# liupei101/AdvMIL

Hardware: AMD Instinct MI355X
Metric: WSI bags/sec (full G+D step) (higher is better)
Workload: dtype bf16x3 (fp32 operands split hi+lo, 3 bf16 MFMAs per product, fp32 accumulate; fp32 storage); 1 GPU; ABMIL+AdvMIL(RLIP prj discriminator), 8192-patch x 1024 fp32 bags (BASELINE.json configs[1] shape; fp32 storage, bf16x3 split arithmetic: >= the bf16 the config names, within 2e-5 of the fp32 reference); gen_updates=1, distinct_resident_bags_per_gpu=64, parallelism=bag-parallel dp1, dropout=shipped rates, launch=hipGraph replay (4 captured bag groups)

## Files before the change

### advmil_amd/_lib.py

```python
import ctypes
import os
from ctypes import c_float, c_int, c_int32, c_int64, c_size_t, c_uint64, c_void_p

LIB_PATH = os.environ.get("ADVMIL_HIP_LIB") or os.path.join(os.path.dirname(os.path.abspath(__file__)), "libadvmil_hip.so")


class HipLibraryMissing(RuntimeError):
    pass


class AdvmilHipError(RuntimeError):
    pass


class Epilogue(ctypes.Structure):
    _fields_ = [("bias", c_void_p), ("act0", c_int), ("act1", c_int), ("act_split", c_int), ("drop_p", c_float),
                ("seed", c_void_p), ("stream_id", c_uint64), ("rowv", c_void_p), ("colv", c_void_p), ("rowseg", c_void_p),
                ("maskref", c_void_p), ("ldmask", c_int), ("mask_scale", c_float), ("accumulate", c_int),
                ("alpha", c_float), ("a_hi", c_void_p), ("a_lo", c_void_p), ("b_hi", c_void_p), ("b_lo", c_void_p),
                ("c_hi", c_void_p), ("c_lo", c_void_p), ("gate_wc", c_void_p), ("gate_out", c_void_p), ("gate_np", c_int),
                ("rng_row", c_void_p), ("c2", c_void_p), ("ldc2", c_int64), ("n_split", c_int64), ("bias2", c_void_p), ("colsum", c_void_p), ("maskbits", c_void_p), ("ldbits", c_int64),
                ("gate_bits_a", c_void_p), ("gate_bits_b", c_void_p), ("ldgbits", c_int64), ("c_rows_pair32", c_int)]


class DenseLayer(ctypes.Structure):
    _fields_ = [("W", c_void_p), ("bias", c_void_p), ("dW", c_void_p), ("dbias", c_void_p), ("y", c_void_p), ("K", c_int), ("N", c_int),
                ("act", c_int), ("drop_p", c_float), ("stream_id", c_uint64)]


TAIL_MAXL = 3


class DTail(ctypes.Structure):
    _fields_ = [("B", c_int), ("nx", c_int), ("ny", c_int), ("prj_src", c_int), ("xin", c_void_p), ("tin", c_void_p),
                ("x", DenseLayer * TAIL_MAXL), ("y", DenseLayer * TAIL_MAXL), ("u", c_void_p), ("w_prj", c_void_p), ("b_prj", c_void_p),
                ("dw_prj", c_void_p), ("db_prj", c_void_p), ("seed", c_void_p), ("rng_row", c_void_p), ("out", c_void_p),
                ("dout", c_void_p), ("dxin", c_void_p), ("dtin", c_void_p), ("du", c_void_p)]


class GemmTnCall(ctypes.Structure):
    _fields_ = [("M", c_int64), ("N", c_int64), ("K", c_int64), ("A", c_void_p), ("lda", c_int64), ("B", c_void_p), ("ldb", c_int64),
                ("C", c_void_p), ("ldc", c_int64), ("accumulate", ctypes.c_int32)]


class GHead(ctypes.Structure):
    _fields_ = [("B", ctypes.c_int32), ("d0", ctypes.c_int32), ("d1", ctypes.c_int32), ("d2", ctypes.c_int32), ("noise_mode", ctypes.c_int32),
                ("out_act", ctypes.c_int32), ("x", c_void_p), ("ldx", c_int64), ("Wr", c_void_p), ("br", c_void_p), ("W0", c_void_p),
                ("b0", c_void_p), ("W1", c_void_p), ("b1", c_void_p), ("p1", c_float), ("p2", c_float), ("seed", c_void_p),
                ("sid1", c_uint64), ("sid2", c_uint64), ("sid_noise", c_uint64), ("rng_row", c_void_p), ("noise", c_void_p),
                ("hs", c_void_p), ("h2", c_void_p), ("pred", c_void_p), ("dpred", c_void_p), ("dx", c_void_p), ("lddx", c_int64),
                ("dWr", c_void_p), ("dbr", c_void_p), ("dW0", c_void_p), ("db0", c_void_p), ("dW1", c_void_p), ("db1", c_void_p),
                ("ws", c_void_p), ("ws_bytes", c_size_t)]


SIGNATURES = {
    "advmil_version": (c_int, []),
    "advmil_gemm_f32_workspace_bytes": (c_size_t, [c_int64, c_int64, c_int]),
    "advmil_gemm_f32": (c_int, [c_int, c_int, c_int64, c_int64, c_int64, c_void_p, c_int64, c_void_p, c_int64, c_void_p,
                                c_int64, ctypes.POINTER(Epilogue), c_int, c_void_p, c_size_t, c_void_p]),
    "advmil_split_planes": (c_int, [c_void_p, c_int64, c_void_p, c_void_p, c_void_p]),
    "advmil_stage_bag": (c_int, [c_void_p, c_void_p, c_size_t, c_void_p, c_void_p, c_void_p, c_void_p, c_size_t, c_void_p]),
    "advmil_gate_interleave": (c_int, [c_void_p, c_void_p, c_void_p, c_void_p, c_int, c_void_p, c_void_p, c_void_p, c_void_p, c_int, c_void_p]),
    "advmil_gate_partial_sum": (c_int, [c_void_p, c_int, c_void_p, c_int64, c_void_p, c_void_p]),
    "advmil_gemm_f32_gate_blocks": (c_int, [c_int, c_int64]),
    "advmil_gemm_f32_colsum_rows": (c_int64, [c_int, c_int64, c_int64]),
    "advmil_merge_partials": (c_int, [c_void_p, c_int, c_int64, c_int64, c_void_p, c_int, c_void_p]),
    "advmil_set_gemm_mode": (c_int, [c_int]),
    "advmil_get_gemm_mode": (c_int, []),
    "advmil_gemm_f32_plan": (c_int, [c_int64, c_int64, c_int64, ctypes.POINTER(c_int), ctypes.POINTER(c_int)]),
    "advmil_gemm_f32_plan_layout": (c_int, [c_int, c_int, c_int64, c_int64, c_int64, ctypes.POINTER(c_int), ctypes.POINTER(c_int)]),
    "advmil_gemm_f32_plan_planes": (c_int, [c_int, c_int, c_int64, c_int64, c_int64, ctypes.POINTER(c_int)]),
    "advmil_gemm_f32_plan_tn_planes": (c_int, [c_int64, c_int64, c_int64, ctypes.POINTER(c_int), ctypes.POINTER(c_int)]),
    "advmil_gemm_f32_tiled": (c_int, [c_int, c_int, c_int64, c_int64, c_int64, c_void_p, c_int64, c_void_p, c_int64, c_void_p,
                                      c_int64, ctypes.POINTER(Epilogue), c_int, c_int, c_void_p, c_size_t, c_void_p]),
    "advmil_mha_fwd": (c_int, [c_void_p, c_void_p, c_int64, c_int, c_int, c_int, c_void_p, c_int64, c_float, c_void_p, c_uint64,
                               c_void_p, c_void_p, c_void_p, c_void_p]),
    "advmil_mha_fwd_lse": (c_int, [c_void_p, c_void_p, c_int64, c_int, c_int, c_int, c_void_p, c_int64, c_float, c_void_p, c_uint64,
                                   c_void_p, c_void_p, c_void_p, c_void_p]),
    "advmil_mha_bwd_workspace_bytes": (c_size_t, [c_int64, c_int, c_int]),
    "advmil_mha_bwd": (c_int, [c_void_p, c_void_p, c_void_p, c_void_p, c_void_p, c_int64, c_int, c_int, c_int, c_void_p, c_int64,
                               c_float, c_void_p, c_uint64, c_void_p, c_void_p, c_void_p, c_size_t, c_void_p]),
    "advmil_mha_bwd1_workspace_bytes": (c_size_t, [c_int64, c_int, c_int, c_int64]),
    "advmil_mha_bwd1": (c_int, [c_void_p, c_void_p, c_void_p, c_void_p, c_void_p, c_int64, c_int, c_int, c_int, c_void_p, c_int64,
                                c_float, c_void_p, c_uint64, c_void_p, c_void_p, c_void_p, c_size_t, c_void_p]),
    "advmil_add_dropout_ln_fwd": (c_int, [c_void_p, c_void_p, c_void_p, c_void_p, c_float, c_int64, c_int64, c_float, c_void_p,
                                          c_uint64, c_void_p, c_void_p, c_void_p, c_void_p, c_void_p, c_void_p, c_void_p, c_void_p]),
    "advmil_add_dropout_ln_bwd_workspace_bytes": (c_size_t, [c_int64, c_int64]),
    "advmil_add_dropout_ln_bwd": (c_int, [c_void_p, c_void_p, c_void_p, c_void_p, c_void_p, c_int64, c_int64, c_float, c_void_p,
                                          c_uint64, c_void_p, c_void_p, c_void_p, c_void_p, c_void_p, c_int, c_void_p, c_size_t,
                                          c_void_p]),
    "advmil_gate_score_fwd": (c_int, [c_void_p, c_void_p, c_void_p, c_float, c_void_p, c_uint64, c_uint64, c_int64, c_int64,
                                      c_void_p, c_void_p, c_void_p]),
    "advmil_softmax_pool_workspace_bytes": (c_size_t, [c_int64, c_int64, c_int]),
    "advmil_softmax_pool_fwd": (c_int, [c_void_p, c_void_p, c_int64, c_int64, c_int64, c_int, c_void_p, c_int64, c_void_p,
                                        c_void_p, c_void_p, c_size_t, c_void_p]),
    "advmil_softmax_pool_mean_workspace_bytes": (c_size_t, [c_int64, c_int64, c_int]),
    "advmil_softmax_pool_mean_fwd": (c_int, [c_void_p, c_void_p, c_int64, c_int64, c_int64, c_int, c_void_p, c_int64, c_void_p,
                                             c_void_p, c_void_p, c_void_p, c_size_t, c_void_p]),
    "advmil_softmax_pool_bwd": (c_int, [c_void_p, c_void_p, c_void_p, c_void_p, c_int64, c_int64, c_int64, c_int, c_void_p,
                                        c_int64, c_void_p, c_void_p, c_size_t, c_void_p]),
    "advmil_softmax_pool_fwd_planes": (c_int, [c_void_p, c_void_p, c_void_p, c_int64, c_int64, c_int64, c_int, c_void_p, c_int64, c_void_p,
                                               c_void_p, c_void_p, c_size_t, c_void_p]),
    "advmil_softmax_pool_bwd_planes": (c_int, [c_void_p, c_void_p, c_void_p, c_void_p, c_void_p, c_int64, c_int64, c_int64, c_int, c_void_p,
                                               c_int64, c_void_p, c_void_p, c_size_t, c_void_p]),
    "advmil_dropout_planes": (c_int, [c_void_p, c_void_p, c_int64, c_int64, c_float, c_void_p, c_uint64, c_void_p, c_void_p, c_void_p, c_void_p,
                                      c_float, c_uint64, c_uint64, c_void_p, c_void_p, c_void_p]),
    "advmil_gate_bwd_workspace_bytes": (c_size_t, [c_int64, c_int64]),
    "advmil_gate_bwd": (c_int, [c_void_p, c_void_p, c_void_p, c_float, c_void_p, c_uint64, c_uint64, c_int64, c_int64,
                                c_void_p, c_void_p, c_void_p, c_void_p, c_int, c_void_p, c_void_p, c_void_p, c_int, c_void_p, c_size_t,
                                c_void_p]),
    "advmil_colsum_workspace_bytes": (c_size_t, [c_int64, c_int64]),
    "advmil_act_dropout_bwd": (c_int, [c_void_p, c_void_p, c_int, c_float, c_void_p, c_uint64, c_int64, c_int64, c_void_p,
                                       c_void_p, c_int, c_void_p, c_void_p, c_void_p, c_void_p, c_void_p, c_size_t, c_void_p]),
    "advmil_colsum": (c_int, [c_void_p, c_int64, c_int64, c_void_p, c_int, c_void_p, c_size_t, c_void_p]),
    "advmil_ln_relu_mean16_fwd": (c_int, [c_void_p, c_void_p, c_void_p, c_float, c_int64, c_int64, c_void_p, c_void_p,
                                          c_void_p, c_void_p, c_void_p, c_int, c_void_p]),
    "advmil_ln_relu_mean16_bwd_workspace_bytes": (c_size_t, [c_int64, c_int64]),
    "advmil_ln_relu_mean16_bwd": (c_int, [c_void_p, c_void_p, c_void_p, c_void_p, c_void_p, c_void_p, c_int64, c_int64,
                                          c_void_p, c_void_p, c_void_p, c_int, c_void_p, c_void_p, c_void_p, c_int, c_void_p, c_size_t, c_void_p]),
    "advmil_ln_relu_fwd": (c_int, [c_void_p, c_void_p, c_void_p, c_float, c_int64, c_int64, c_void_p, c_void_p, c_void_p, c_void_p]),
    "advmil_ln_relu_bwd_workspace_bytes": (c_size_t, [c_int64, c_int64]),
    "advmil_ln_relu_bwd": (c_int, [c_void_p, c_void_p, c_void_p, c_void_p, c_void_p, c_void_p, c_int64, c_int64, c_void_p,
                                   c_void_p, c_void_p, c_int, c_void_p, c_size_t, c_void_p]),
    "advmil_genconv_fwd": (c_int, [c_void_p, c_void_p, c_void_p, c_void_p, c_float, c_int64, c_int64, c_void_p, c_void_p,
                                   c_void_p, c_void_p]),
    "advmil_genconv_bwd_workspace_bytes": (c_size_t, [c_int64, c_int64]),
    "advmil_genconv_bwd": (c_int, [c_void_p, c_void_p, c_void_p, c_void_p, c_void_p, c_void_p, c_void_p, c_float, c_int64,
                                   c_int64, c_void_p, c_void_p, c_void_p, c_size_t, c_void_p]),
    "advmil_adam_step": (c_int, [c_void_p, c_void_p, c_void_p, c_void_p, c_void_p, c_int64, c_float, c_float, c_float,
                                 c_float, c_float, c_float, c_void_p, c_void_p, c_void_p, c_int, c_void_p, c_int, c_void_p]),
    "advmil_adam_blocks": (c_int, [c_int64]),
    "advmil_step_seed_tick": (c_int, [c_void_p, c_void_p, c_void_p, c_uint64, c_void_p]),
    "advmil_abs_sum": (c_int, [c_void_p, c_int64, c_void_p, c_void_p, c_size_t, c_void_p]),
    "advmil_abs_sum_workspace_bytes": (c_size_t, [c_int64]),
    "advmil_uniform_fill": (c_int, [c_void_p, c_int64, c_void_p, c_uint64, c_void_p, c_int64, c_void_p]),
    "advmil_dropout_apply": (c_int, [c_void_p, c_void_p, c_int64, c_float, c_void_p, c_uint64, c_void_p, c_int64, c_void_p]),
    "advmil_seed_advance": (c_int, [c_void_p, c_uint64, c_void_p]),
    "advmil_seg_scale_rows": (c_int, [c_void_p, c_void_p, c_void_p, c_int64, c_int64, c_void_p, c_void_p]),
    "advmil_stamp_clock": (c_int, [c_void_p, c_void_p]),
    "advmil_clock_rate_khz": (c_int64, []),
    "advmil_small_linear_fwd": (c_int, [c_void_p, c_int64, c_void_p, c_void_p, c_int, c_int, c_int, c_int, c_float, c_void_p, c_uint64,
                                        c_void_p, c_void_p, c_void_p]),
    "advmil_small_linear_bwd_workspace_bytes": (c_size_t, [c_int, c_int]),
    "advmil_small_linear_bwd": (c_int, [c_void_p, c_void_p, c_void_p, c_int64, c_void_p, c_int, c_int, c_int, c_int, c_float, c_void_p,
                                        c_uint64, c_void_p, c_void_p, c_int, c_void_p, c_int, c_void_p, c_int64, c_void_p, c_size_t, c_void_p]),
    "advmil_skinny_linear_fwd": (c_int, [c_void_p, c_void_p, c_void_p, c_int, c_int, c_int, c_int, c_void_p, c_void_p]),
    "advmil_skinny_linear_bwd": (c_int, [c_void_p, c_void_p, c_void_p, c_void_p, c_int, c_int, c_int, c_int, c_void_p, c_void_p,
                                         c_void_p, c_int, c_void_p]),
    "advmil_prj_head_fwd": (c_int, [c_void_p, c_void_p, c_void_p, c_void_p, c_void_p, c_int, c_int, c_void_p, c_void_p]),
    "advmil_prj_head_bwd": (c_int, [c_void_p, c_void_p, c_void_p, c_void_p, c_void_p, c_int, c_int, c_void_p, c_void_p, c_void_p, c_void_p,
                                    c_void_p, c_int, c_void_p]),
    "advmil_gan_d_loss": (c_int, [c_void_p, c_int, c_void_p, c_void_p, c_int, c_int, c_float, c_float, c_void_p, c_void_p, c_void_p, c_void_p]),
    "advmil_gan_g_loss": (c_int, [c_void_p, c_void_p, c_void_p, c_void_p, c_void_p, c_int, c_float, c_float, c_int, c_float, c_float,
                                  c_float, c_void_p, c_void_p, c_void_p, c_void_p]),
    "advmil_dx_chain_fwd": (c_int, [c_void_p, c_int64, c_int, c_void_p, c_void_p, c_void_p, c_void_p, c_void_p, c_void_p, c_void_p, c_void_p,
                                    c_void_p, c_void_p, c_void_p, c_float, c_float, c_void_p, c_uint64, c_uint64, c_uint64, c_void_p, c_void_p,
                                    c_void_p, c_void_p, c_void_p, c_void_p]),
    "advmil_dx_chain_bwd_workspace_bytes": (c_size_t, [c_int64, c_int]),
    "advmil_dx_chain_prep": (c_int, [c_void_p, c_void_p, c_void_p, c_int, c_void_p, c_void_p, c_void_p, c_void_p, c_void_p, c_void_p, c_void_p]),
    "advmil_dx_chain_bwd": (c_int, [c_int64, c_int, c_void_p, c_void_p, c_void_p, c_void_p, c_void_p, c_void_p, c_void_p, c_void_p, c_void_p,
                                    c_void_p, c_float, c_float, c_void_p, c_uint64, c_uint64, c_void_p, c_void_p, c_void_p, c_void_p, c_void_p,
                                    c_void_p, c_void_p, c_void_p, c_void_p, c_void_p, c_void_p, c_void_p, c_void_p, c_void_p, c_void_p, c_void_p,
                                    c_void_p, c_size_t, c_void_p]),
    "advmil_dtail_fwd": (c_int, [ctypes.POINTER(DTail), c_void_p]),
    "advmil_dtail_bwd": (c_int, [ctypes.POINTER(DTail), c_void_p]),
    "advmil_gemm_tn_group_workspace_bytes": (c_size_t, [ctypes.POINTER(GemmTnCall), c_int]),
    "advmil_gemm_tn_group": (c_int, [ctypes.POINTER(GemmTnCall), c_int, c_void_p, c_size_t, c_void_p]),
    "advmil_ghead_workspace_bytes": (c_size_t, [c_int, c_int, c_int, c_int]),
    "advmil_ghead_fwd": (c_int, [ctypes.POINTER(GHead), c_void_p]),
    "advmil_ghead_bwd": (c_int, [ctypes.POINTER(GHead), c_void_p]),
    "advmil_defer_sums": (c_int, [c_void_p, c_int]),
    "advmil_flush_sums": (c_int, [c_void_p]),
    "advmil_pending_sums": (c_int, [c_void_p]),
    "advmil_cindex_counts": (c_int, [c_void_p, c_void_p, c_void_p, c_int64, c_float, c_void_p, c_void_p]),
}

_lib = None
DEFAULT_GEMM_MODE = "bf16x3"
_GEMM_MODES = {"exact": 0, "f32": 0, "bf16x3": 1, "split": 1}


def lib():
    global _lib
    if _lib is None:
        if not os.path.exists(LIB_PATH):
# ... 21 lines not shown
```

### advmil_amd/csrc/pool.hip

```cpp
#include <cstdlib>
#include "common.h"
#include "bf16split.h"
#include "sumq.h"
#include "../../include/advmil_hip.h"

#define ROWS_PER_BLOCK 32
static inline int rows_per_block(int64_t rows) {
  int64_t r = (rows + 1023) / 1024;
  r = (r + 31) / 32 * 32;
  if (r < ROWS_PER_BLOCK) r = ROWS_PER_BLOCK;
  if (r > 512) r = 512;
  return (int)r;
}

struct RowColMap {
  int cols4, rpp, c4, r;
  bool active;
};
__device__ __forceinline__ RowColMap make_map(int64_t D) {
  RowColMap m;
  m.cols4 = (int)(D >> 2);
  m.rpp = 256 / m.cols4;
  if (m.rpp < 1) m.rpp = 1;
  m.c4 = threadIdx.x % m.cols4;
// ... 211 lines not shown
                                                           int64_t ldh, int64_t N, int64_t D,
                                                           const int64_t* __restrict__ seg_ptr,
                                                           const float* __restrict__ stats, float* __restrict__ A,
                                                           float* __restrict__ partial, int rpb) {
  __shared__ __attribute__((aligned(16))) float red[1024];
  const RowColMap m = make_map(D);
  const int b = blockIdx.y;
  int64_t beg, end;
  seg_range(seg_ptr, b, N, beg, end);
  const float mx = stats[2 * b], inv = stats[2 * b + 1];
  const int64_t r0 = beg + (int64_t)blockIdx.x * rpb;
  float4 acc = make_float4(0.f, 0.f, 0.f, 0.f);
  if (m.active) {
    for (int r = m.r; r < rpb; r += m.rpp) {
      const int64_t n = r0 + r;
      if (n >= end) break;
      const float w = hw_exp(s[n] - mx) * inv;
      if (m.c4 == 0) A[n] = w;
      const float4 v = *reinterpret_cast<const float4*>(h + n * ldh + m.c4 * 4);
      acc.x += w * v.x; acc.y += w * v.y; acc.z += w * v.z; acc.w += w * v.w;
    }
  }
  const float4 t = reduce_rows(acc, m, red);
  if (m.active && m.r == 0)
    *reinterpret_cast<float4*>(partial + ((int64_t)b * gridDim.x + blockIdx.x) * D + m.c4 * 4) = t;
}

__global__ __launch_bounds__(256) void pool_partial8_kernel(const float* __restrict__ s, const float* __restrict__ h, int64_t ldh,
                                                            int64_t N, int64_t D, const int64_t* __restrict__ seg_ptr,
                                                            const float* __restrict__ stats, float* __restrict__ A,
                                                            float* __restrict__ partial, int rpb) {
  __shared__ __attribute__((aligned(16))) float red[2048];
  const int cols8 = (int)(D >> 3), rpp = 256 / cols8;
  const int c8 = threadIdx.x % cols8, rl = threadIdx.x / cols8;
  const int b = blockIdx.y;
  int64_t beg, end;
  seg_range(seg_ptr, b, N, beg, end);
  const float mx = stats[2 * b], inv = stats[2 * b + 1];
  const int64_t r0 = beg + (int64_t)blockIdx.x * rpb;
  float acc[8];
#pragma unroll
  for (int j = 0; j < 8; ++j) acc[j] = 0.f;
  if (rl < rpp) {
#pragma unroll 4
    for (int r = rl; r < rpb; r += rpp) {
      const int64_t n = r0 + r;
      const bool ok = n < end;
      const int64_t nn = ok ? n : beg;
      const float w = ok ? hw_exp(s[nn] - mx) * inv : 0.f;
      const float4 v0 = *reinterpret_cast<const float4*>(h + nn * ldh + c8 * 8);
      const float4 v1 = *reinterpret_cast<const float4*>(h + nn * ldh + c8 * 8 + 4);
      if (ok && c8 == 0) A[n] = w;
      acc[0] += w * v0.x; acc[1] += w * v0.y; acc[2] += w * v0.z; acc[3] += w * v0.w;
      acc[4] += w * v1.x; acc[5] += w * v1.y; acc[6] += w * v1.z; acc[7] += w * v1.w;
    }
    float* dst = red + (int64_t)rl * D + c8 * 8;
    *reinterpret_cast<float4*>(dst) = make_float4(acc[0], acc[1], acc[2], acc[3]);
    *reinterpret_cast<float4*>(dst + 4) = make_float4(acc[4], acc[5], acc[6], acc[7]);
  }
  __syncthreads();
  if ((int)threadIdx.x < (int)(D >> 2)) {
    float4 t = make_float4(0.f, 0.f, 0.f, 0.f);
    for (int q = 0; q < rpp; ++q) {
      const float4 v = *reinterpret_cast<const float4*>(red + (int64_t)q * D + threadIdx.x * 4);
      t.x += v.x; t.y += v.y; t.z += v.z; t.w += v.w;
    }
    *reinterpret_cast<float4*>(partial + ((int64_t)b * gridDim.x + blockIdx.x) * D + threadIdx.x * 4) = t;
  }
}

__device__ __forceinline__ void planes8(const bf16raw* __restrict__ hi, const bf16raw* __restrict__ lo, int64_t off, float4& v0, float4& v1) {
  const uint4 a = *reinterpret_cast<const uint4*>(hi + off);
  const uint4 b = *reinterpret_cast<const uint4*>(lo + off);
  v0.x = __uint_as_float(a.x << 16) + __uint_as_float(b.x << 16);
  v0.y = __uint_as_float(a.x & 0xffff0000u) + __uint_as_float(b.x & 0xffff0000u);
  v0.z = __uint_as_float(a.y << 16) + __uint_as_float(b.y << 16);
  v0.w = __uint_as_float(a.y & 0xffff0000u) + __uint_as_float(b.y & 0xffff0000u);
  v1.x = __uint_as_float(a.z << 16) + __uint_as_float(b.z << 16);
  v1.y = __uint_as_float(a.z & 0xffff0000u) + __uint_as_float(b.z & 0xffff0000u);
  v1.z = __uint_as_float(a.w << 16) + __uint_as_float(b.w << 16);
  v1.w = __uint_as_float(a.w & 0xffff0000u) + __uint_as_float(b.w & 0xffff0000u);
}

template <bool MEAN, bool PL = false>
__global__ __launch_bounds__(256) void pool_partial8_online_kernel(const float* __restrict__ s, const float* __restrict__ h, int64_t ldh,
                                                                   int64_t N, int64_t D, const int64_t* __restrict__ seg_ptr,
                                                                   float* __restrict__ partial, float* __restrict__ pstats, int rpb,
                                                                   float* __restrict__ mpartial, const bf16raw* __restrict__ hlo = nullptr) {
  __shared__ __attribute__((aligned(16))) float red[2048];
  __shared__ float wts[512];
  __shared__ float wred[8];
  const int cols8 = (int)(D >> 3), rpp = 256 / cols8;
  const int c8 = threadIdx.x % cols8, rl = threadIdx.x / cols8;
  const int tid = threadIdx.x, lane = tid & 63, w = tid >> 6;
  const int b = blockIdx.y;
  int64_t beg, end;
  seg_range(seg_ptr, b, N, beg, end);
  const int64_t r0 = beg + (int64_t)blockIdx.x * rpb;
  float* pst = pstats + ((int64_t)b * gridDim.x + blockIdx.x) * 2;
  float* prow = partial + ((int64_t)b * gridDim.x + blockIdx.x) * D;
  float* mrow = MEAN ? mpartial + ((int64_t)b * gridDim.x + blockIdx.x) * D : nullptr;
  if (r0 >= end) {
    if (tid < (int)(D >> 2)) {
      *reinterpret_cast<float4*>(prow + tid * 4) = make_float4(0.f, 0.f, 0.f, 0.f);
      if (MEAN) *reinterpret_cast<float4*>(mrow + tid * 4) = make_float4(0.f, 0.f, 0.f, 0.f);
    }
    if (tid == 0) { pst[0] = -INFINITY; pst[1] = 0.f; }
    return;
  }
  float mx = -INFINITY;
  for (int r = tid; r < rpb; r += 256) {
    const int64_t n = r0 + r;
    const float v = n < end ? s[n] : -INFINITY;
    wts[r] = v;
    mx = fmaxf(mx, v);
  }
  mx = wave_max(mx);
  if (lane == 0) wred[w] = mx;
  __syncthreads();
  mx = fmaxf(fmaxf(wred[0], wred[1]), fmaxf(wred[2], wred[3]));
  float ls = 0.f;
  for (int r = tid; r < rpb; r += 256) {
    const float e = (r0 + r < end) ? hw_exp(wts[r] - mx) : 0.f;
    wts[r] = e;
    ls += e;
  }
  ls = wave_sum(ls);
  if (lane == 0) wred[4 + w] = ls;
  __syncthreads();
  if (tid == 0) { pst[0] = mx; pst[1] = (wred[4] + wred[5]) + (wred[6] + wred[7]); }
  float acc[8], macc[8];
#pragma unroll
  for (int j = 0; j < 8; ++j) { acc[j] = 0.f; macc[j] = 0.f; }
  if (rl < rpp) {
#pragma unroll 4
    for (int r = rl; r < rpb; r += rpp) {
      const int64_t n = r0 + r;
      const int64_t nn = n < end ? n : beg;
      const float wgt = wts[r];
      float4 v0, v1;
      if constexpr (PL) {
        planes8(reinterpret_cast<const bf16raw*>(h), hlo, nn * ldh + c8 * 8, v0, v1);
      } else {
        v0 = *reinterpret_cast<const float4*>(h + nn * ldh + c8 * 8);
        v1 = *reinterpret_cast<const float4*>(h + nn * ldh + c8 * 8 + 4);
      }
      acc[0] += wgt * v0.x; acc[1] += wgt * v0.y; acc[2] += wgt * v0.z; acc[3] += wgt * v0.w;
      acc[4] += wgt * v1.x; acc[5] += wgt * v1.y; acc[6] += wgt * v1.z; acc[7] += wgt * v1.w;
      if (MEAN) {
        const float one = n < end ? 1.f : 0.f;
        macc[0] += one * v0.x; macc[1] += one * v0.y; macc[2] += one * v0.z; macc[3] += one * v0.w;
        macc[4] += one * v1.x; macc[5] += one * v1.y; macc[6] += one * v1.z; macc[7] += one * v1.w;
      }
    }
    float* dst = red + (int64_t)rl * D + c8 * 8;
    *reinterpret_cast<float4*>(dst) = make_float4(acc[0], acc[1], acc[2], acc[3]);
    *reinterpret_cast<float4*>(dst + 4) = make_float4(acc[4], acc[5], acc[6], acc[7]);
  }
  __syncthreads();
  if (tid < (int)(D >> 2)) {
    float4 t = make_float4(0.f, 0.f, 0.f, 0.f);
    for (int q = 0; q < rpp; ++q) {
      const float4 v = *reinterpret_cast<const float4*>(red + (int64_t)q * D + tid * 4);
      t.x += v.x; t.y += v.y; t.z += v.z; t.w += v.w;
    }
    *reinterpret_cast<float4*>(prow + tid * 4) = t;
  }
  if (MEAN) {
    __syncthreads();
    if (rl < rpp) {
      float* dst = red + (int64_t)rl * D + c8 * 8;
      *reinterpret_cast<float4*>(dst) = make_float4(macc[0], macc[1], macc[2], macc[3]);
      *reinterpret_cast<float4*>(dst + 4) = make_float4(macc[4], macc[5], macc[6], macc[7]);
    }
    __syncthreads();
    if (tid < (int)(D >> 2)) {
      float4 t = make_float4(0.f, 0.f, 0.f, 0.f);
      for (int q = 0; q < rpp; ++q) {
        const float4 v = *reinterpret_cast<const float4*>(red + (int64_t)q * D + tid * 4);
        t.x += v.x; t.y += v.y; t.z += v.z; t.w += v.w;
      }
      *reinterpret_cast<float4*>(mrow + tid * 4) = t;
    }
  }
}

#define POOL_ONLINE_MAX_NBLK 2048
__global__ __launch_bounds__(256) void pool_merge_online_kernel(const float* __restrict__ partial, const float* __restrict__ pstats, int nblk,
                                                                int64_t D, const float* __restrict__ s, int64_t N,
                                                                const int64_t* __restrict__ seg_ptr, float* __restrict__ pooled,
                                                                float* __restrict__ A, float* __restrict__ stats,
                                                                const float* __restrict__ mpartial = nullptr, float* __restrict__ mean = nullptr) {
  __shared__ float sc[POOL_ONLINE_MAX_NBLK];
  __shared__ float red[16][17];
  __shared__ float wred[8];
  const int tid = threadIdx.x, lane = tid & 63, w = tid >> 6;
  const int b = blockIdx.y;
  const float* pst = pstats + (int64_t)b * nblk * 2;
  float mx = -INFINITY;
  for (int j = tid; j < nblk; j += 256) mx = fmaxf(mx, pst[2 * j]);
  mx = wave_max(mx);
  if (lane == 0) wred[w] = mx;
  __syncthreads();
  const float M = fmaxf(fmaxf(wred[0], wred[1]), fmaxf(wred[2], wred[3]));
  float ls = 0.f;
  for (int j = tid; j < nblk; j += 256) {
    const float mj = pst[2 * j];
    const float c = mj == -INFINITY ? 0.f : hw_exp(mj - M);
    sc[j] = c;
    ls += pst[2 * j + 1] * c;
  }
  ls = wave_sum(ls);
  if (lane == 0) wred[4 + w] = ls;
  __syncthreads();
  const float inv = hw_rcp((wred[4] + wred[5]) + (wred[6] + wred[7]));
  if (blockIdx.x == 0 && tid == 0 && stats) { stats[2 * b] = M; stats[2 * b + 1] = inv; }
  const int cl = tid & 15, rl = tid >> 4;
  const int64_t c = (int64_t)blockIdx.x * 16 + cl;
  const float* pp = partial + (int64_t)b * nblk * D;
  float sv[4] = {0.f, 0.f, 0.f, 0.f};
  if (c < D) {
    int j = rl;
    for (; j + 48 < nblk; j += 64) {
#pragma unroll
      for (int u = 0; u < 4; ++u) sv[u] += pp[(int64_t)(j + 16 * u) * D + c] * sc[j + 16 * u];
    }
    for (; j < nblk; j += 16) sv[0] += pp[(int64_t)j * D + c] * sc[j];
  }
  red[rl][cl] = (sv[0] + sv[1]) + (sv[2] + sv[3]);
  __syncthreads();
  if (rl == 0 && c < D) {
    float t = 0.f;
#pragma unroll
    for (int r = 0; r < 16; ++r) t += red[r][cl];
    pooled[(int64_t)b * D + c] = t * inv;
  }
  int64_t beg, end;
  seg_range(seg_ptr, b, N, beg, end);
  if (mean) {
    __syncthreads();
    const float* mp = mpartial + (int64_t)b * nblk * D;
    float mv[4] = {0.f, 0.f, 0.f, 0.f};
    if (c < D) {
      int j = rl;
      for (; j + 48 < nblk; j += 64) {
#pragma unroll
        for (int u = 0; u < 4; ++u) mv[u] += mp[(int64_t)(j + 16 * u) * D + c];
      }
      for (; j < nblk; j += 16) mv[0] += mp[(int64_t)j * D + c];
    }
    red[rl][cl] = (mv[0] + mv[1]) + (mv[2] + mv[3]);
    __syncthreads();
    if (rl == 0 && c < D) {
      float t = 0.f;
#pragma unroll
      for (int r = 0; r < 16; ++r) t += red[r][cl];
      mean[(int64_t)b * D + c] = end > beg ? t / (float)(end - beg) : 0.f;
    }
  }
  for (int64_t n = beg + (int64_t)blockIdx.x * 256 + tid; n < end; n += (int64_t)gridDim.x * 256) A[n] = hw_exp(s[n] - M) * inv;
}

static inline int64_t pool_nblk(int64_t max_len) { const int r = rows_per_block(max_len); return (max_len + r - 1) / r; }

extern "C" size_t advmil_softmax_pool_workspace_bytes(int64_t max_len, int64_t D, int nseg) {
  if (nseg < 1) nseg = 1;
  const int64_t a = 4 * (int64_t)nseg + (int64_t)nseg * pool_nblk(max_len) * (D + 2);
  const int64_t b = 4 + (int64_t)nseg * ((max_len + 3) / 4);
  return (size_t)(a > b ? a : b) * sizeof(float);
}

static int softmax_pool_fwd_impl(const float* s, const float* h, int64_t ldh, int64_t N, int64_t D, int nseg, const int64_t* seg_ptr,
                                 int64_t max_len, float* A, float* pooled, float* mean, void* ws, size_t ws_bytes, hipStream_t stream,
                                 const bf16raw* hlo = nullptr);

extern "C" int advmil_softmax_pool_fwd(const float* s, const float* h, int64_t ldh, int64_t N, int64_t D, int nseg,
                                       const int64_t* seg_ptr, int64_t max_len, float* A, float* pooled, void* ws,
                                       size_t ws_bytes, advmil_stream_t stream_) {
  return softmax_pool_fwd_impl(s, h, ldh, N, D, nseg, seg_ptr, max_len, A, pooled, nullptr, ws, ws_bytes, (hipStream_t)stream_);
}

extern "C" int advmil_softmax_pool_fwd_planes(const float* s, const void* h_hi, const void* h_lo, int64_t ldh, int64_t N, int64_t D, int nseg,
                                              const int64_t* seg_ptr, int64_t max_len, float* A, float* pooled, void* ws,
                                              size_t ws_bytes, advmil_stream_t stream_) {
  if (!h_hi || !h_lo) return ADVMIL_EINVAL;
  return softmax_pool_fwd_impl(s, (const float*)h_hi, ldh, N, D, nseg, seg_ptr, max_len, A, pooled, nullptr, ws, ws_bytes, (hipStream_t)stream_,
                               (const bf16raw*)h_lo);
}

static inline size_t pool_mean_offset_bytes(int64_t max_len, int64_t D, int nseg) {
  return (advmil_softmax_pool_workspace_bytes(max_len, D, nseg) + 15) / 16 * 16;
}

extern "C" size_t advmil_softmax_pool_mean_workspace_bytes(int64_t max_len, int64_t D, int nseg) {
  if (nseg < 1) nseg = 1;
  return pool_mean_offset_bytes(max_len, D, nseg) + (size_t)((int64_t)nseg * pool_nblk(max_len) * D) * sizeof(float);
}

extern "C" int advmil_softmax_pool_mean_fwd(const float* s, const float* h, int64_t ldh, int64_t N, int64_t D, int nseg,
                                            const int64_t* seg_ptr, int64_t max_len, float* A, float* pooled, float* mean, void* ws,
                                            size_t ws_bytes, advmil_stream_t stream_) {
  if (!mean) return ADVMIL_EINVAL;
  return softmax_pool_fwd_impl(s, h, ldh, N, D, nseg, seg_ptr, max_len, A, pooled, mean, ws, ws_bytes, (hipStream_t)stream_);
}

static int softmax_pool_fwd_impl(const float* s, const float* h, int64_t ldh, int64_t N, int64_t D, int nseg, const int64_t* seg_ptr,
                                 int64_t max_len, float* A, float* pooled, float* mean, void* ws, size_t ws_bytes, hipStream_t stream,
                                 const bf16raw* hlo) {
  if (!s || !h || !A || !pooled || !ws || N <= 0 || D <= 0 || (D & 3) || D > 1024 || (ldh & 3)) return ADVMIL_EINVAL;
  if (ldh < D || ((uintptr_t)h & 15)) return ADVMIL_EINVAL;
  if (hlo && (((uintptr_t)hlo & 15) || (D & 7) || (ldh & 7) || D < 16 || mean)) return ADVMIL_EINVAL;
  if (!seg_ptr && nseg > 1) return ADVMIL_EINVAL;
  if (!seg_ptr) { nseg = 1; max_len = N; }
  if (nseg < 1 || max_len <= 0 || max_len > N) return ADVMIL_EINVAL;
  if (ws_bytes < (mean ? advmil_softmax_pool_mean_workspace_bytes(max_len, D, nseg) : advmil_softmax_pool_workspace_bytes(max_len, D, nseg)))
    return ADVMIL_EWORKSPACE;
  float* stats = (float*)ws;
  float* partial = stats + 4 * nseg;
  const int nblk = (int)pool_nblk(max_len);
  if ((D & 7) == 0 && D >= 16 && nblk <= POOL_ONLINE_MAX_NBLK) {
    float* pstats = partial + (int64_t)nseg * nblk * D;
    if (mean) {
      float* mpartial = (float*)ws + pool_mean_offset_bytes(max_len, D, nseg) / sizeof(float);
      hipLaunchKernelGGL((pool_partial8_online_kernel<true, false>), dim3(nblk, nseg), dim3(256), 0, stream, s, h, ldh, N, D, seg_ptr, partial, pstats,
                         rows_per_block(max_len), mpartial, (const bf16raw*)nullptr);
      ADVMIL_LAUNCH_CHECK();
      hipLaunchKernelGGL(pool_merge_online_kernel, dim3((unsigned)((D + 15) / 16), nseg), dim3(256), 0, stream, partial, pstats, nblk, D, s,
                         N, seg_ptr, pooled, A, stats, (const float*)mpartial, mean);
      ADVMIL_LAUNCH_CHECK();
      return ADVMIL_OK;
    }
    if (hlo)
      hipLaunchKernelGGL((pool_partial8_online_kernel<false, true>), dim3(nblk, nseg), dim3(256), 0, stream, s, h, ldh, N, D, seg_ptr, partial,
                         pstats, rows_per_block(max_len), (float*)nullptr, hlo);
    else
      hipLaunchKernelGGL((pool_partial8_online_kernel<false, false>), dim3(nblk, nseg), dim3(256), 0, stream, s, h, ldh, N, D, seg_ptr, partial,
                         pstats, rows_per_block(max_len), (float*)nullptr, (const bf16raw*)nullptr);
    ADVMIL_LAUNCH_CHECK();
    hipLaunchKernelGGL(pool_merge_online_kernel, dim3((unsigned)((D + 15) / 16), nseg), dim3(256), 0, stream, partial, pstats, nblk, D, s,
                       N, seg_ptr, pooled, A, stats, (const float*)nullptr, (float*)nullptr);
    ADVMIL_LAUNCH_CHECK();
    return ADVMIL_OK;
  }
  if (mean || hlo) return ADVMIL_EINVAL;
  hipLaunchKernelGGL(softmax_stats_kernel, dim3(nseg), dim3(1024), 0, stream, s, N, seg_ptr, stats);
  ADVMIL_LAUNCH_CHECK();
  if ((D & 7) == 0 && D >= 16)
    hipLaunchKernelGGL(pool_partial8_kernel, dim3(nblk, nseg), dim3(256), 0, stream, s, h, ldh, N, D, seg_ptr, stats, A, partial,
                       rows_per_block(max_len));
  else
    hipLaunchKernelGGL(pool_partial_kernel, dim3(nblk, nseg), dim3(256), 0, stream, s, h, ldh, N, D, seg_ptr, stats, A, partial,
                       rows_per_block(max_len));
  ADVMIL_LAUNCH_CHECK();
  hipLaunchKernelGGL(colsum_merge_kernel, dim3((unsigned)((D + 15) / 16), nseg), dim3(256), 0, stream, partial, nblk, D, D, pooled,
                     0, (int64_t)nblk * D, D);
  ADVMIL_LAUNCH_CHECK();
  return ADVMIL_OK;
}

#define PBD_ROWS 4
template <bool PL>
__global__ __launch_bounds__(256) void pool_bwd_dot_kernel(const float* __restrict__ dp, const float* __restrict__ dA,
                                                           const float* __restrict__ A, const float* __restrict__ h,
                                                           int64_t ldh, int64_t N, int64_t D,
                                                           const int64_t* __restrict__ seg_ptr, float* __restrict__ t,
                                                           float* __restrict__ partial, const bf16raw* __restrict__ hlo) {
  __shared__ float red[4];
  const int lane = threadIdx.x & 63, w = threadIdx.x >> 6;
  const int b = blockIdx.y;
  int64_t beg, end;
  seg_range(seg_ptr, b, N, beg, end);
  const int64_t n0 = beg + ((int64_t)blockIdx.x * 4 + w) * PBD_ROWS;
  const float* dpb = dp + (int64_t)b * D;
  float acc[PBD_ROWS];
#pragma unroll
  for (int rr = 0; rr < PBD_ROWS; ++rr) acc[rr] = 0.f;
  if (PL && n0 < end) {
    const int nch = (int)(D >> 3), items = PBD_ROWS * nch;
    for (int g = lane; g < items; g += 64) {
      const int rr = g / nch, ch = g - rr * nch;
      if (n0 + rr < end) {
        float4 v0, v1;
        planes8(reinterpret_cast<const bf16raw*>(h), hlo, (n0 + rr) * ldh + ch * 8, v0, v1);
        const float4 a0 = *reinterpret_cast<const float4*>(dpb + ch * 8), a1 = *reinterpret_cast<const float4*>(dpb + ch * 8 + 4);
        const float d = a0.x * v0.x + a0.y * v0.y + a0.z * v0.z + a0.w * v0.w + a1.x * v1.x + a1.y * v1.y + a1.z * v1.z + a1.w * v1.w;
#pragma unroll
        for (int k = 0; k < PBD_ROWS; ++k) acc[k] += (k == rr) ? d : 0.f;
      }
    }
  } else if (n0 < end) {
    if ((D & 3) == 0 && (ldh & 3) == 0) {
      const float4* d4 = reinterpret_cast<const float4*>(dpb);
      for (int64_t q = lane; q < (D >> 2); q += 64) {
        const float4 a = d4[q];
        float4 v[PBD_ROWS];
#pragma unroll
        for (int rr = 0; rr < PBD_ROWS; ++rr)
          v[rr] = (n0 + rr < end) ? reinterpret_cast<const float4*>(h + (n0 + rr) * ldh)[q] : make_float4(0.f, 0.f, 0.f, 0.f);
#pragma unroll
        for (int rr = 0; rr < PBD_ROWS; ++rr) acc[rr] += a.x * v[rr].x + a.y * v[rr].y + a.z * v[rr].z + a.w * v[rr].w;
      }
    } else {
      for (int64_t j = lane; j < D; j += 64) {
        const float a = dpb[j];
#pragma unroll
        for (int rr = 0; rr < PBD_ROWS; ++rr)
          if (n0 + rr < end) acc[rr] += a * h[(n0 + rr) * ldh + j];
      }
    }
  }
  float contrib = 0.f;
#pragma unroll
  for (int rr = 0; rr < PBD_ROWS; ++rr) {
    const int64_t n = n0 + rr;
    float s = wave_sum(acc[rr]);
    if (n < end) {
      if (dA) s += dA[n];
      if (lane == 0) t[n] = s;
      contrib += A[n] * s;
    }
  }
  if (lane == 0) red[w] = contrib;
  __syncthreads();
  if (threadIdx.x == 0) partial[(int64_t)b * gridDim.x + blockIdx.x] = red[0] + red[1] + red[2] + red[3];
}

__global__ __launch_bounds__(256) void pool_bwd_ds_kernel(const float* __restrict__ A, const float* __restrict__ partial,
// ... 104 lines not shown
    return ADVMIL_EINVAL;
  if ((((uintptr_t)in_hi | (uintptr_t)in_lo | (uintptr_t)out_hi | (uintptr_t)out_lo) & 15) || ((uintptr_t)bits & 3)) return ADVMIL_EINVAL;
  int64_t blocks = (M * (N >> 3) + 255) / 256;
  if (blocks > 8192) blocks = 8192;
  hipLaunchKernelGGL(dropout_planes_kernel, dim3((unsigned)blocks), dim3(256), 0, (hipStream_t)stream_, (const bf16raw*)in_hi, (const bf16raw*)in_lo,
                     M, N, drop_p, seed, stream_id, rng_row, (bf16raw*)out_hi, (bf16raw*)out_lo, (uint8_t*)bits, gate_p, gate_stream_a,
                     gate_stream_b, (uint8_t*)gate_bits_a, (uint8_t*)gate_bits_b);
  ADVMIL_LAUNCH_CHECK();
  return ADVMIL_OK;
}

__global__ __launch_bounds__(256) void seg_scale_rows_kernel(const float* __restrict__ dpooled, const float* __restrict__ A,
                                                             const int32_t* __restrict__ rowseg, int64_t N, int64_t D,
                                                             float* __restrict__ dh) {
  const int64_t q4 = D >> 2, total = N * q4;
  for (int64_t e = (int64_t)blockIdx.x * 256 + threadIdx.x; e < total; e += (int64_t)gridDim.x * 256) {
    const int64_t n = e / q4, c = (e % q4) * 4;
    const float a = A[n];
    const float4 v = *reinterpret_cast<const float4*>(dpooled + (int64_t)(rowseg ? rowseg[n] : 0) * D + c);
    *reinterpret_cast<float4*>(dh + n * D + c) = make_float4(a * v.x, a * v.y, a * v.z, a * v.w);
  }
}
extern "C" int advmil_seg_scale_rows(const float* dpooled, const float* A, const int32_t* rowseg, int64_t N, int64_t D, float* dh,
                                     advmil_stream_t stream_) {
  if (!dpooled || !A || !dh || N <= 0 || D <= 0 || (D & 3) || (((uintptr_t)dpooled | (uintptr_t)dh) & 15)) return ADVMIL_EINVAL;
  int64_t blocks = (N * (D >> 2) + 255) / 256;
  if (blocks > 4096) blocks = 4096;
  hipLaunchKernelGGL(seg_scale_rows_kernel, dim3((unsigned)blocks), dim3(256), 0, (hipStream_t)stream_, dpooled, A, rowseg, N, D, dh);
  ADVMIL_LAUNCH_CHECK();
  return ADVMIL_OK;
}

__global__ __launch_bounds__(256) void gate_interleave_kernel(const float* __restrict__ Wa, const float* __restrict__ Wb,
                                                              const float* __restrict__ ba, const float* __restrict__ bb, int D,
                                                              float* __restrict__ Wi, bf16raw* __restrict__ hi, bf16raw* __restrict__ lo,
                                                              float* __restrict__ bi, int pair32) {
  const int q4 = D >> 2;
  const int64_t total = (int64_t)2 * D * q4;
  for (int64_t e = (int64_t)blockIdx.x * 256 + threadIdx.x; e < total; e += (int64_t)gridDim.x * 256) {
    const int r = (int)(e / q4), c = (int)(e % q4) * 4;
    const int br = pair32 ? ((r >> 5) & 1) : (r & 1), j = pair32 ? (((r >> 6) << 5) | (r & 31)) : (r >> 1);
    const float* src = br ? Wb : Wa;
    const float4 v = *reinterpret_cast<const float4*>(src + (int64_t)j * D + c);
    *reinterpret_cast<float4*>(Wi + (int64_t)r * D + c) = v;
    if (hi) {
      uint2 hh, ll;
      split4(v, hh, ll);
      *reinterpret_cast<uint2*>(hi + (int64_t)r * D + c) = hh;
      *reinterpret_cast<uint2*>(lo + (int64_t)r * D + c) = ll;
    }
  }
  if (blockIdx.x == 0)
    for (int r = threadIdx.x; r < 2 * D; r += 256) {
      const int br = pair32 ? ((r >> 5) & 1) : (r & 1), j = pair32 ? (((r >> 6) << 5) | (r & 31)) : (r >> 1);
      bi[r] = br ? bb[j] : ba[j];
    }
}
__global__ __launch_bounds__(256) void gate_partial_sum_kernel(const float* __restrict__ partial, int np, const float* __restrict__ bc,
                                                               int64_t N, float* __restrict__ s) {
  const float b = bc ? bc[0] : 0.f;
  for (int64_t n = (int64_t)blockIdx.x * 256 + threadIdx.x; n < N; n += (int64_t)gridDim.x * 256) {
    float a = 0.f;
    for (int j = 0; j < np; ++j) a += partial[n * np + j];
    s[n] = a + b;
  }
}
extern "C" int advmil_gate_interleave(const float* Wa, const float* Wb, const float* ba, const float* bb, int D, float* Wi, void* Wi_hi,
                                      void* Wi_lo, float* bi, int pair32, advmil_stream_t stream_) {
  if (!Wa || !Wb || !ba || !bb || !Wi || !bi || D <= 0 || (D & 3) || ((Wi_hi != nullptr) != (Wi_lo != nullptr))) return ADVMIL_EINVAL;
  if (pair32 && (D & 31)) return ADVMIL_EINVAL;
  if (((uintptr_t)Wa & 15) || ((uintptr_t)Wb & 15) || ((uintptr_t)Wi & 15) || ((uintptr_t)Wi_hi & 7) || ((uintptr_t)Wi_lo & 7)) return ADVMIL_EINVAL;
  int64_t blocks = ((int64_t)2 * D * (D >> 2) + 255) / 256;
  if (blocks > 1024) blocks = 1024;
  hipLaunchKernelGGL(gate_interleave_kernel, dim3((unsigned)blocks), dim3(256), 0, (hipStream_t)stream_, Wa, Wb, ba, bb, D, Wi,
                     (bf16raw*)Wi_hi, (bf16raw*)Wi_lo, bi, pair32);
  ADVMIL_LAUNCH_CHECK();
  return ADVMIL_OK;
}
extern "C" int advmil_gate_partial_sum(const float* partial, int np, const float* bc, int64_t N, float* s, advmil_stream_t stream_) {
  if (!partial || !s || np <= 0 || N <= 0) return ADVMIL_EINVAL;
  int64_t blocks = (N + 255) / 256;
  if (blocks > 2048) blocks = 2048;
  hipLaunchKernelGGL(gate_partial_sum_kernel, dim3((unsigned)blocks), dim3(256), 0, (hipStream_t)stream_, partial, np, bc, N, s);
  ADVMIL_LAUNCH_CHECK();
  return ADVMIL_OK;
}

__global__ __launch_bounds__(256) void gate_bwd_kernel(const float* __restrict__ ab, const float* __restrict__ ds,
                                                       const float* __restrict__ wc, float p, const uint64_t* seed,
                                                       uint64_t stream_a, uint64_t stream_b, int64_t N, int64_t D,
                                                       float* __restrict__ dG, float* __restrict__ partial, int rpb,
                                                       const int64_t* __restrict__ rng_row, bf16raw* __restrict__ g_hi,
                                                       bf16raw* __restrict__ g_lo, int pair32) {
  __shared__ __attribute__((aligned(16))) float red[1024];
  const RowColMap m = make_map(D);
  const int64_t oa = pair32 ? (int64_t)(((m.c4 * 4) >> 5) << 6) + ((m.c4 * 4) & 31) : (int64_t)m.c4 * 4;
  const int64_t ob = pair32 ? oa + 32 : D + (int64_t)m.c4 * 4;
  const bool drop = seed && p > 0.f;
  uint64_t ka = 0, kb = 0;
  float inv = 1.f;
  if (drop) {
    const uint64_t sd = *seed;
    ka = rng_key(sd, stream_a); kb = rng_key(sd, stream_b); inv = hw_rcp(1.f - p);
  }
  const int64_t r0 = (int64_t)blockIdx.x * rpb;
  float4 s_wc = make_float4(0.f, 0.f, 0.f, 0.f), s_a = s_wc, s_b = s_wc;
  float s_ds = 0.f;
  if (m.active) {
    const float4 w4 = *reinterpret_cast<const float4*>(wc + m.c4 * 4);
    const float wv[4] = {w4.x, w4.y, w4.z, w4.w};
    for (int r = m.r; r < rpb; r += m.rpp) {
      const int64_t n = r0 + r;
      if (n >= N) break;
      const float d = ds[n];
      if (m.c4 == 0) s_ds += d;
      const float4 a4 = *reinterpret_cast<const float4*>(ab + n * 2 * D + oa);
      const float4 b4 = *reinterpret_cast<const float4*>(ab + n * 2 * D + ob);
      const float av[4] = {a4.x, a4.y, a4.z, a4.w}, bv[4] = {b4.x, b4.y, b4.z, b4.w};
      float ga[4], gb[4], gw[4];
      float fa4[4] = {1.f, 1.f, 1.f, 1.f}, fb4[4] = {1.f, 1.f, 1.f, 1.f};
      if (drop) {
        const uint64_t idx = (uint64_t)((rng_row ? rng_row[n] : n) * D + m.c4 * 4);
        rng_keep4(ka, idx, p, inv, fa4);
        rng_keep4(kb, idx, p, inv, fb4);
      }
#pragma unroll
      for (int q = 0; q < 4; ++q) {
        const float fa = fa4[q], fb = fb4[q];
        const float ad = av[q] * fa, bd = bv[q] * fb;
        gw[q] = d * ad * bd;
        ga[q] = d * wv[q] * bd * fa * (1.f - av[q] * av[q]);
        gb[q] = d * wv[q] * ad * fb * bv[q] * (1.f - bv[q]);
      }
      if (dG) {
        *reinterpret_cast<float4*>(dG + n * 2 * D + oa) = make_float4(ga[0], ga[1], ga[2], ga[3]);
        *reinterpret_cast<float4*>(dG + n * 2 * D + ob) = make_float4(gb[0], gb[1], gb[2], gb[3]);
      }
      if (g_hi) {
        uint2 hh, ll;
        split4(make_float4(ga[0], ga[1], ga[2], ga[3]), hh, ll);
        *reinterpret_cast<uint2*>(g_hi + n * 2 * D + oa) = hh;
        *reinterpret_cast<uint2*>(g_lo + n * 2 * D + oa) = ll;
        split4(make_float4(gb[0], gb[1], gb[2], gb[3]), hh, ll);
        *reinterpret_cast<uint2*>(g_hi + n * 2 * D + ob) = hh;
        *reinterpret_cast<uint2*>(g_lo + n * 2 * D + ob) = ll;
      }
      s_wc.x += gw[0]; s_wc.y += gw[1]; s_wc.z += gw[2]; s_wc.w += gw[3];
      s_a.x += ga[0]; s_a.y += ga[1]; s_a.z += ga[2]; s_a.w += ga[3];
      s_b.x += gb[0]; s_b.y += gb[1]; s_b.z += gb[2]; s_b.w += gb[3];
    }
  }
  float* prow = partial + (int64_t)blockIdx.x * (3 * D + 4);
  float4 t = reduce_rows(s_wc, m, red);
  if (m.active && m.r == 0) *reinterpret_cast<float4*>(prow + m.c4 * 4) = t;
  t = reduce_rows(s_a, m, red);
  if (m.active && m.r == 0) *reinterpret_cast<float4*>(prow + D + m.c4 * 4) = t;
  t = reduce_rows(s_b, m, red);
  if (m.active && m.r == 0) *reinterpret_cast<float4*>(prow + 2 * D + m.c4 * 4) = t;
  __syncthreads();
  if (m.active && m.c4 == 0) red[m.r] = s_ds;
  __syncthreads();
  if (threadIdx.x == 0) {
    float q = 0.f;
    for (int r = 0; r < m.rpp; ++r) q += red[r];
    prow[3 * D] = q;
  }
// ... 763 lines not shown
```

### advmil_amd/graphed.py

```python
import os

import torch

from . import ops


CLEAR_IN_ADAM = os.environ.get("ADVMIL_CLEAR_IN_ADAM", "1") != "0"


class GraphedStep:
    def __init__(self, handler, xs, ys, ys_host, mode="wlabel", label_visible_mask=None, warmup=2, force_segments=False,
                 capture_collectives=None, plan=None, keep_warmup=False, pool=None, site_base=None):
        self.keep_warmup, self.warm_out = bool(keep_warmup), None
        self.pool = pool
        self.site_base = site_base
        self.force_segments = force_segments
        self.h = handler
        self.wait_events = []
        self.captured_collectives = False
        if capture_collectives is None:
            capture_collectives = os.environ.get("ADVMIL_GRAPH_COLLECTIVES", "1") != "0"
        dp = handler.dp
        want = bool(capture_collectives and dp.enabled and (dp.world > 1 or getattr(dp, "force", False)) and not force_segments
                    and torch.distributed.get_backend(dp.group) == "nccl")
# ... 1 lines not shown
        self.xs, self.ys = xs, ys
        self.plan = plan if plan is not None else handler._plan(xs, ys, mode, label_visible_mask, ys_host)
        self.lrs = self._lrs()
        self.segments = []
        self.logs = None
        self._capture(warmup)

    def _agree(self, flag):
        dp = self.h.dp
        if not (dp.enabled and dp.world > 1):
            return bool(flag)
        t = torch.tensor([1.0 if flag else 0.0], device=self.h.device)
        torch.distributed.all_reduce(t, op=torch.distributed.ReduceOp.MIN, group=dp.group)
        return bool(float(t.item()) > 0.5)

    def _whole(self):
        self._seg_disc()
        self.h._reduce_d()
        self._seg_gfwd()
        self._seg_mid()
        self.h._reduce_g()
        self._seg_end()

    def _lrs(self):
        return (self.h.optimizerG.param_groups[0]["lr"], self.h.optimizerD.param_groups[0]["lr"])

    def _seg_disc(self):
        self.preds, self.fakes = self.h._disc_backward(0, self.xs, self.ys, self.plan)

    def _seg_gfwd(self):
        self.h._gen_forward(self.xs, self.plan)

    def _seg_mid(self):
        self.h._log_d()
        self.h.optimizerD.step(tick=False, clear_grad=CLEAR_IN_ADAM)
        self.h._gen_finish(0, self.xs, self.ys, self.plan)

    def _seg_end(self):
        self.h._log_g()
        self.h.optimizerG.step(tick=False, abs_partial=self.h._abs_partial, clear_grad=CLEAR_IN_ADAM)
        ops.step_seed_tick(self.h.optimizerG.step_t, self.h.rng.seed, 1, step2=self.h.optimizerD.step_t)

    def _eager(self):
        self._seg_disc()
        pend = self.h.dp.allreduce_async(self.h.optimizerD.flat_grad, self.h._st_d[0])
        self._seg_gfwd()
        for w in pend:
            w.wait()
        self._seg_mid()
        self.h._reduce_g()
        self._seg_end()

    def _capture(self, warmup):
        h = self.h
        saved = list(h.history)
        cur = torch.cuda.current_stream()
        side = torch.cuda.Stream()
        side.wait_stream(cur)
        with torch.cuda.stream(side):
            for _ in range(warmup):
                if self.site_base is not None:
                    h.rng.counter = self.site_base
                self._eager()
            if self.keep_warmup and warmup:
                self.warm_out = (torch.cat(self.preds, dim=0).detach().clone(), torch.cat(self.fakes, dim=0).detach().clone())
        cur.wait_stream(side)
        torch.cuda.synchronize()
        if self.keep_warmup:
            saved = list(h.history)
        del h.history[:]
        pool = self.pool if self.pool is not None else torch.cuda.graph_pool_handle()
        for opt in (h.optimizerD, h.optimizerG):
            opt.capture_assumes_clean = CLEAR_IN_ADAM
        try:
            self._capture_graphs(pool)
        finally:
            for opt in (h.optimizerD, h.optimizerG):
                opt.capture_assumes_clean = False
        self.logs = list(h.history)
        h.history[:] = saved
        self._st_d, self._st_g = h._st_d, h._st_g

    def _capture_graphs(self, pool):
        h = self.h
        if self.site_base is not None:
            h.rng.counter = self.site_base
        if self._want_captured:
            ok = True
            try:
                g = torch.cuda.CUDAGraph()
                with torch.cuda.graph(g, pool=pool, capture_error_mode="thread_local"):
                    self._whole()
            except Exception:
                ok = False
                torch.cuda.synchronize()
            if self._agree(ok):
                self.segments.append(g)
                self.captured_collectives = True
            else:
                self._want_captured = False
                del h.history[:]
        if not self.segments:
            if h.dp.world > 1 or self.force_segments or (h.dp.enabled and getattr(h.dp, "force", False)):
                parts = (self._seg_disc, self._seg_gfwd, self._seg_mid, self._seg_end)
            else:
                parts = (lambda: (self._seg_disc(), self._seg_gfwd(), self._seg_mid(), self._seg_end()),)
            for fn in parts:
                g = torch.cuda.CUDAGraph()
                with torch.cuda.graph(g, pool=pool, capture_error_mode="thread_local"):
                    fn()
                self.segments.append(g)

    def replay(self):
        if self._lrs() != self.lrs:
            self.segments, self.lrs = [], self._lrs()
            self._capture(0)
        segs = self.segments
        if CLEAR_IN_ADAM:
            for opt in (self.h.optimizerD, self.h.optimizerG):
                if not opt.grad_is_clean():
                    opt.flat_grad.zero_()
                opt.mark_grad_dirty()
        if len(segs) == 1:
            segs[0].replay()
            if CLEAR_IN_ADAM:
                self.h.optimizerD.mark_grad_clean(); self.h.optimizerG.mark_grad_clean()
            return
        segs[0].replay()
        self.h._st_d, self.h._st_g = self._st_d, self._st_g
        pend = self.h.dp.allreduce_async(self.h.optimizerD.flat_grad, self._st_d[0])
        segs[1].replay()
        stamp = self.stamp_waits
        if stamp:
            ev = [torch.cuda.Event(enable_timing=True) for _ in range(4)]
            ev[0].record()
        for w in pend:
            w.wait()
        if stamp:
            ev[1].record()
        segs[2].replay()
        if stamp:
            ev[2].record()
        self.h._reduce_g()
        if stamp:
            ev[3].record()
            self.wait_events = [(ev[0], ev[1]), (ev[2], ev[3])]
        segs[3].replay()
        if CLEAR_IN_ADAM:
            self.h.optimizerD.mark_grad_clean(); self.h.optimizerG.mark_grad_clean()

    stamp_waits = False

    def exposed_allreduce_ms(self):
        return tuple(a.elapsed_time(b) for a, b in self.wait_events)
```

### advmil_amd/model/model_handler.py

```python
import os
import os.path as osp
from functools import partial
from types import SimpleNamespace

import torch

from .. import ops
from ..loss.utils import fake_generator_loss, real_fake_loss, real_fake_terms, recon_loss, recon_terms
from ..optim import FlatAdam, create_optimizer
from ..ingest import BagCache, SlabStager, bag_fingerprint, x_store_dtype
from ..parallel import BagParallel
from ..utils.func import agg_tensor, seed_everything, sparse_key, sparse_str
from .backbone import load_backbone
from .GANSurv import Discriminator, Generator, PrjDiscriminator
from .model_utils import init_weights


def _check_configs(cfg):
    assert cfg["task"] in ("cont_gansurv",), "HIP path covers task=cont_gansurv (the only task in the shipped config)"
    assert cfg["batch_size"] == 1, "batch_size must be 1 (one WSI per forward)"
    assert cfg["loss_netD"] in ("bce", "hinge", "wasserstein")
    assert cfg["disc_type"] in ("prj", "cat")
    assert cfg["gen_out_scale"] in ("sigmoid", "exp", "none", None)

# ... 503 lines not shown
    def _slab_build(self, xs, pad=0):
        return MyHandler._slab_build_static(xs, getattr(self, "resident_planes", True), pad)

    @staticmethod
    def _bags(t, plan, stacked=False):
        if t is None or not getattr(plan, "pad", 0):
            return t
        return t.index_select(0, plan.sel2) if stacked else t[:plan.nb]

    @staticmethod
    def _slab_build_static(xs, resident_planes=True, pad=0):
        x0 = xs[0][0]
        c = x0.shape[-1]
        rows = [x[0].shape[-2] for x in xs]
        ok = all(x[0].is_contiguous() for x in xs)
        if ok:
            st = x0.untyped_storage().data_ptr()
            ptr = x0.data_ptr()
            for x, r in zip(xs, rows):
                if x[0].data_ptr() != ptr or x[0].untyped_storage().data_ptr() != st:
                    ok = False
                    break
                ptr += r * c * x0.element_size()
        if pad and not ok:
            raise RuntimeError("a slab pad needs the bags back to back in the staging slab")
        X = (x0.as_strided((sum(rows) + pad, c), (c, 1), x0.storage_offset()) if ok
             else torch.cat([x[0].reshape(-1, c) for x in xs], dim=0))
        if ops.is_bf16_slab(X):
            return X
        spl = getattr(x0, "_advmil_stager_planes", None) if ok else None
        stale = bool(getattr(x0, "_advmil_fp32_stale", False))
        if spl is not None and spl.hi.shape[0] == X.shape[0] and ops.slab_takes_planes(X.shape[0], c):
            X._advmil_planes = spl
            if stale:
                X._advmil_planes = ops.Planes(spl.hi, spl.lo)
                X._advmil_planes.fp32_stale = True
                X._advmil_fp32_stale = True
            return X
        if stale:
            raise RuntimeError("advmil_amd: a step slab staged as operand planes only cannot be read as fp32 rows (planes missing / not "
                               "back to back / arithmetic mode changed between staging and the step)")
        pls = None if ok else [getattr(x[0], "_advmil_bag_planes", None) for x in xs]
        if (pls and all(p is not None for p in pls) and X.shape[0] >= 4096 and ops.USE_PLANES and ops.get_gemm_mode() == "bf16x3"
                and ops.gemm_plan_planes(X.shape[0], 128, c)):
            xpl = ops.Planes.alloc(tuple(X.shape), X.device)
            torch.cat([p.hi for p in pls], dim=0, out=xpl.hi)
            torch.cat([p.lo for p in pls], dim=0, out=xpl.lo)
            X._advmil_planes = xpl
        else:
            MyHandler._slab_planes_static(X, x0 if ok else None, resident_planes)
        return X

    def _slab_planes(self, X, anchor):
        MyHandler._slab_planes_static(X, anchor, getattr(self, "resident_planes", True))

    @staticmethod
    def _slab_planes_static(X, anchor, resident_planes=True):
        if X.shape[0] < 4096 or not ops.USE_PLANES or ops.get_gemm_mode() != "bf16x3":
            return
        if not ops.SLAB_PLANES_ANY and not ops.gemm_plan_planes(X.shape[0], 128, X.shape[1]):
            return
        if anchor is None or not resident_planes:
            X._advmil_planes = ops.split_planes(X)
            return
        cache = anchor.__dict__.setdefault("_advmil_slab_planes", {})
        ent = cache.get(X.shape[0])
        if ent is None or ent[0] != X._version:
            ent = (X._version, ops.split_planes(X, out=None if ent is None else ent[1]))
            cache[X.shape[0]] = ent
        X._advmil_planes = ent[1]

    @staticmethod
    def _stack_noise(noise):
        if noise is None:
            return None
        return [torch.cat([nb[j] for nb in noise], dim=0) for j in range(len(noise[0]))]

    def _prefill_first_layers(self, X):
        return MyHandler._prefill_static(self.netG, self.netD, self.bcb, X)

    @staticmethod
    def _prefill_static(netG, netD, bcb, X):
        bb = netG.backbone
        if bcb == "abmil" and hasattr(bb, "attention_net"):
            fc = bb.attention_net[0]
            l1 = (fc.weight, fc.bias, "relu", True)
        elif bcb == "patch" and hasattr(bb, "patch_embedding_layer") and hasattr(bb.patch_embedding_layer, "conv"):
            cv = bb.patch_embedding_layer.conv
            l1 = (cv.weight, cv.bias, "none", False)
        else:
            return False
        emb = getattr(getattr(netD, "net_pair_one", None), "embedding", None)
        if emb is None or not hasattr(emb, "conv"):
            return False
        return ops.prefill_two_layers(X, l1, (emb.conv.weight, emb.conv.bias, "none", False))

    def _gen_features(self, X, plan, xs):
        exts = [x[1] for x in xs] if self.bcb in ("cluster", "graph") else None
        pad = getattr(plan, "pad", 0)
        if self.bcb == "cluster" and all(torch.is_tensor(e) and not e.is_cuda for e in exts):
            ids = plan.__dict__.get("_cluster_ids")
            if ids is None:
                n = sum(int(e.numel()) for e in exts)
                buf = torch.zeros(n + pad, dtype=exts[0].dtype, pin_memory=True)
                torch.cat([e.reshape(-1) for e in exts], out=buf[:n])
                ids = plan._cluster_ids = buf.to(self.device, non_blocking=True)
            exts = [ids]
        elif exts is not None and pad:
            exts = exts + [torch.zeros(pad, dtype=exts[0].dtype, device=exts[0].device)]
        return self._bags(self.netG.features_multi(X, plan.seg, exts), plan)

    def _disc_backward(self, i_batch, xs, ys, plan, noise=None):
        self._set_mode(self.netD, True)
        self._set_mode(self.netG, False)
        self.rng.rows = plan.rng_rows
        try:
            return self._disc_backward_body(i_batch, xs, ys, plan, noise)
        finally:
            self.rng.rows = None

    def _disc_backward_body(self, i_batch, xs, ys, plan, noise=None):
        self.optimizerD.zero_grad()
        X = self._slab(xs, plan)
        y = plan.y
        self._prefill_first_layers(X)
        ops.MEMO.begin("record", ("G", id(self.netG), getattr(self.optimizerG, "n_updates", 0), plan.token), X)
        try:
            with torch.no_grad():
                pred = self.netG.finish(self._gen_features(X, plan, xs), noise=self._stack_noise(noise),
                                        pred_out=None if plan.t2 is None else plan.t2[:len(xs)])
        finally:
            ops.MEMO.end()
        f_real = f2 = None
        emb = self.netD.embed_rows(X, 2) if plan.n_real > 0 else self.netD.embed_rows(X)
        if plan.n_real > 0:
            nb = len(xs)
            eb2, im2 = self.netD.bag_features_multi(emb, plan.seg16.twice())
            eb2, im2 = self._bags(eb2, plan, True), self._bags(im2, plan, True)
            t2 = plan.t2 if (plan.t2 is not None and pred.data_ptr() == plan.t2.data_ptr()) else torch.cat([pred, plan.y_t], dim=0)
            f2 = self.netD.tail(eb2, im2, t2).view(-1)
            f_fake = f2.detach()[:nb]
        else:
            eb, im = self.netD.bag_features_multi(emb, plan.seg16)
            f_fake = self.netD.tail(self._bags(eb, plan), self._bags(im, plan), pred).view(-1)
        ops.PREFILL.clear()
        ops.DY_PLANES.clear()
        if f2 is not None:
            loss, st = ops.gan_d_loss_stacked(f2, len(xs), plan.real_mask, self.which_loss, plan.n_fake, plan.n_real, root=True)
        else:
            loss, st = ops.gan_d_loss(f_fake, None, None, self.which_loss, plan.n_fake, plan.n_real, root=True)
        try:
            with torch.autograd.set_multithreading_enabled(False), ops.deferred_sums():
                torch.autograd.backward(loss, grad_tensors=self._one())
        finally:
            ops.DY_PLANES.clear()
        self._st_d = (st, plan, i_batch)
        if plan.t2 is not None and pred.data_ptr() == plan.t2.data_ptr() and not torch.cuda.is_current_stream_capturing():
            pred = pred.clone()
        preds = list(pred.split(1, dim=0))
        fakes = list(f_fake.detach().split(1, dim=0))
        return preds, fakes

    def _one(self):
        return self._one_t

    def _reduce_d(self):
        self.dp.allreduce_(self.optimizerD.flat_grad)
        self.dp.allreduce_(self._st_d[0])

    def _log_d(self):
        st, plan, i_batch = self._st_d
        nr, nf = max(plan.n_real, 1), plan.n_fake
        self.log(LazyLog((st,), lambda v: {"train_batch/netD/Loss_D": v[0], "train_batch/netD/D_real": v[1] / nr,
                                           "train_batch/netD/D_fake": v[2] / nf, "i_batch": i_batch}))

    def _disc_apply(self):
        self._reduce_d()
        self._log_d()
# ... 196 lines not shown
```

### advmil_amd/ops.py

```python
import ctypes
import os

import torch

from . import _lib
from ._lib import Epilogue

ACT_NONE, ACT_RELU, ACT_TANH, ACT_SIGMOID = 0, 1, 2, 3
FUSED_WGRAD = True
KERNEL_PROFILE = None
STAMPS = None


class Stamps:

    def __init__(self, device, cap=2048):
        self.buf = torch.zeros(cap, dtype=torch.int64, device=device)
        self.tags = []
        self.khz = int(_lib.lib().advmil_clock_rate_khz()) or 100000

    def mark(self, tag):
        i = len(self.tags)
        if i >= self.buf.numel():
            return
# ... 472 lines not shown
    if accumulate:
        e.accumulate = 1
    e.alpha = float(alpha)
    if a_planes is not None:
        e.a_hi, e.a_lo = a_planes.hi.data_ptr(), a_planes.lo_ptr()
    if b_planes is not None:
        e.b_hi, e.b_lo = b_planes.hi.data_ptr(), b_planes.lo_ptr()
    if c_planes is not None:
        e.c_hi, e.c_lo = c_planes.hi.data_ptr(), c_planes.lo.data_ptr()
    if gate_wc is not None:
        e.gate_wc, e.gate_out, e.gate_np = gate_wc.data_ptr(), gate_out.data_ptr(), npart
        if gate_bits is not None:
            e.gate_bits_a, e.gate_bits_b, e.ldgbits = gate_bits[0].data_ptr(), gate_bits[1].data_ptr(), gate_bits[0].stride(0)
    if c_rows_pair32:
        e.c_rows_pair32 = 1
    if colsum is not None:
        e.colsum = colsum.data_ptr()
    if maskbits is not None:
        e.maskbits, e.ldbits = maskbits.data_ptr(), maskbits.stride(0)
        e.mask_scale = float(mask_scale)
    if splits is None:
        ptile, splits = gemm_plan(M, N, K, a_kc, b_kc)
        if tile == 0:
            tile = ptile
    if accumulate and splits > 1 and _DEFER_KEEP is not None and out is not None and not _is_arena(out):
        splits = 1
    if b_only and not (91 <= tile <= 93) and tile not in (22, 12, 11) and not (tile in (34, 24) and not a_kc and not b_kc):
        tile = 22
    if planes_only_a and a_planes.single and not (82 <= tile <= 86) and tile not in (22, 12, 11):
        tile = 22
    if planes_only_a and a_planes.fp32_stale and not (82 <= tile <= 86) and not (91 <= tile <= 93) and tile not in (22, 12, 11) \
            and not pre_a_tile_ok(tile, a_kc, b_kc, b_planes is not None):
        tile = 22
    if planes_only_a and not (82 <= tile <= 86) and not (91 <= tile <= 93) and not pre_a_tile_ok(tile if tile else gemm_plan(M, N, K, a_kc, b_kc)[0], a_kc, b_kc,
                                                                     b_planes is not None):
        raise ValueError(f"gemm(A=None): tile {tile} has no pre-split-A instantiation for this layout")
    L = _lib.lib()
    wsb = L.advmil_gemm_f32_workspace_bytes(M, N, splits)
    ws = _ws(wsb, A.device) if wsb else None
    prof = KERNEL_PROFILE
    name = None
    if prof is not None or STAMPS is not None:
        name = ("gemm_nt_planes_kernel<%d>" % (tile - 80)) if 82 <= tile <= 84 else "gemm_nt_planes_kernel<4,plain>" if tile == 85 else "gemm_nt_planes_kernel<2,plain>" if tile == 86 else \
            ("gemm_tn_planes_kernel<%d>" % tile) if 91 <= tile <= 93 else \
            "gemm_f32_kernel<%d,%d,%d,%d>" % (bool(a_kc), bool(b_kc), tile // 10, tile % 10)
    if prof is not None:
        e0 = torch.cuda.Event(enable_timing=True)
        e0.record()
    if STAMPS is not None and M * N * K >= (1 << 30):
        _stamp("b", name, (M, N, K, splits), 2.0 * M * N * K)
    _lib.check(L.advmil_gemm_f32_tiled(1 if a_kc else 0, 1 if b_kc else 0, M, N, K, _p(A), lda, _p(B), ldb, _p(out), ldc,
                                       ctypes.byref(e), splits, tile, _p(ws), wsb, _stream()), f"gemm_f32[{M}x{N}x{K}]")
    if STAMPS is not None and M * N * K >= (1 << 30):
        _stamp("e", name, (M, N, K, splits), 2.0 * M * N * K)
    if prof is not None:
        e1 = torch.cuda.Event(enable_timing=True)
        e1.record()
        prof.append((name, (M, N, K, splits), 2.0 * M * N * K, e0, e1))
    if gate_wc is not None and gate_bits is not None:
        return out, gate_out
    return gate_out if gate_wc is not None else out


ATTN_QKV_PLANES = os.environ.get("ADVMIL_ATTN_QKV_PLANES", "1") != "0"
TWO_LAYERS_MIN_TILES = int(os.environ.get("ADVMIL_TWO_LAYERS_MIN_TILES", "256"))
TWO_LAYERS_NARROW = os.environ.get("ADVMIL_TWO_LAYERS_NARROW", "1") != "0"


def gemm_two_layers_tile(M, N1, N2, K):
    if not (get_gemm_mode() == "bf16x3" and USE_PLANES and M >= 4096 and M % 256 == 0 and K % 32 == 0 and K >= 64 and N1 % 32 == 0
            and M * K * 2 < (1 << 32)):
        return 0
    if (N1 + N2) % 256 == 0 and (M // 256) * ((N1 + N2) // 256) >= TWO_LAYERS_MIN_TILES:
        return 85
    if TWO_LAYERS_NARROW and (N1 + N2) % 128 == 0 and N1 % 128 == 0 and (M // 256) * ((N1 + N2) // 128) >= TWO_LAYERS_MIN_TILES:
        return 86
    return 0


def gemm_two_layers_ok(M, N1, N2, K):
    return gemm_two_layers_tile(M, N1, N2, K) != 0


def gemm_two_layers(x, xpl, W1, w1pl, b1, act1, W2, w2pl, b2, act2, emit_planes1=False, y1_planes_only=False):
    M, K = x.shape
    N1, N2 = W1.shape[0], W2.shape[0]

    def pair(pl, N):
        hi, lo = pl.hi.reshape(N, K), pl.lo.reshape(N, K)
        d = (lo.data_ptr() - hi.data_ptr()) // 2
        if hi.untyped_storage().data_ptr() != lo.untyped_storage().data_ptr() or d <= 0 or not hi.is_contiguous() or not lo.is_contiguous():
            return None
        return hi.as_strided((2, N, K), (d, K, 1), hi.storage_offset())
    v1, v2 = pair(w1pl, N1), pair(w2pl, N2)
    if v1 is not None and v2 is not None:
        stk = torch.cat((v1, v2), dim=1)
        wcat = Planes(stk[0], stk[1])
    else:
        wcat = Planes(torch.cat((w1pl.hi.reshape(N1, K), w2pl.hi.reshape(N2, K)), dim=0), torch.cat((w1pl.lo.reshape(N1, K), w2pl.lo.reshape(N2, K)), dim=0))
    dev = x.device
    y1 = _token(M, N1, dev) if y1_planes_only else torch.empty(M, N1, dtype=torch.float32, device=dev)
    y2 = torch.empty(M, N2, dtype=torch.float32, device=dev)
    cpl = None
    if emit_planes1 or y1_planes_only:
        cpl = Planes.alloc((M, N1), dev)
    e = Epilogue()
    e.bias = None if b1 is None else b1.data_ptr()
    e.bias2 = None if b2 is None else b2.data_ptr()
    e.act0, e.act1, e.act_split = act1, act2, N1
    e.alpha = 1.0
    e.a_hi, e.a_lo = xpl.hi.data_ptr(), xpl.lo_ptr()
    e.b_hi, e.b_lo = wcat.hi.data_ptr(), wcat.lo.data_ptr()
    if cpl is not None:
        e.c_hi, e.c_lo = cpl.hi.data_ptr(), cpl.lo.data_ptr()
    e.c2, e.ldc2, e.n_split = y2.data_ptr(), N2, N1
    prof = KERNEL_PROFILE
    if prof is not None:
        e0 = torch.cuda.Event(enable_timing=True)
        e0.record()
    _stamp("b", f"gemm_nt_planes_kernel<4,two layers,{N1}>", (M, N1 + N2, K, 1), 2.0 * M * (N1 + N2) * K)
    _lib.check(_lib.lib().advmil_gemm_f32_tiled(1, 1, M, N1 + N2, K, _p(x), x.stride(0), _p(W1), K, None if y1_planes_only else _p(y1), N1,
                                                ctypes.byref(e), 1, gemm_two_layers_tile(M, N1, N2, K), None, 0, _stream()),
               f"gemm_two_layers[{M}x({N1}+{N2})x{K}]")
    if cpl is not None:
        cpl.fp32_stale = bool(y1_planes_only)
    _stamp("e", f"gemm_nt_planes_kernel<4,two layers,{N1}>", (M, N1 + N2, K, 1), 2.0 * M * (N1 + N2) * K)
    if prof is not None:
        e1 = torch.cuda.Event(enable_timing=True)
        e1.record()
        prof.append((f"gemm_nt_planes_kernel<4,two layers,{N1}>", (M, N1 + N2, K, 1), 2.0 * M * (N1 + N2) * K, e0, e1))
    return y1, y2, cpl


def gate_score(ab, wc, bc, N, D, p=0.0, seed=None, stream_a=0, stream_b=0, rng_row=None):
    s = torch.empty(N, dtype=torch.float32, device=ab.device)
    sd = seed if p > 0.0 else None
    _lib.check(_lib.lib().advmil_gate_score_fwd(_p(ab), _p(wc), _p(bc), p, _p(sd), stream_a, stream_b, N, D, _p(s),
                                                _p(rng_row if sd is not None else None), _stream()), "gate_score_fwd")
    return s


class Segments:

    def __init__(self, lens, device):
        import numpy as np
        self.lens = [int(v) for v in lens]
        self.nseg = len(self.lens)
        self.total = sum(self.lens)
        self.max_len = max(self.lens)
        self.device = torch.device(device)
        offs = [0]
        for v in self.lens:
            offs.append(offs[-1] + v)
        self.offsets = offs
        nb = (8 * (self.nseg + 1) + 15) // 16 * 16
        host = torch.empty(nb + 4 * self.total, dtype=torch.uint8, pin_memory=self.device.type == "cuda")
        hv = host.numpy()
        hv[:8 * (self.nseg + 1)].view(np.int64)[:] = offs
        hv[nb:].view(np.int32)[:] = np.repeat(np.arange(self.nseg, dtype=np.int32), self.lens)
        buf = host.to(self.device, non_blocking=True)
        self._host, self._buf = host, buf
        self.ptr = buf[:8 * (self.nseg + 1)].view(torch.int64)
        self.rowseg = buf[nb:].view(torch.int32)
        self._div = {}

    @property
    def rowseg_long(self):
        if "long" not in self._div:
            self._div["long"] = self.rowseg.to(torch.long)
        return self._div["long"]

    def div(self, k):
        if k not in self._div:
            assert all(v % k == 0 for v in self.lens)
            self._div[k] = Segments([v // k for v in self.lens], self.device)
        return self._div[k]

    def twice(self):
        if "x2" not in self._div:
            self._div["x2"] = Segments(self.lens + self.lens, self.device)
        return self._div["x2"]

    def uniform(self, rows):
        key = ("u", rows)
        if key not in self._div:
            self._div[key] = Segments([rows] * self.nseg, self.device)
        return self._div[key]


def softmax_pool(s, h, N, D, seg=None, hpl=None):
    L = _lib.lib()
    nseg = 1 if seg is None else seg.nseg
    mlen = N if seg is None else seg.max_len
    A = torch.empty(N, dtype=torch.float32, device=h.device)
    pooled = torch.empty(nseg, D, dtype=torch.float32, device=h.device)
    wsb = L.advmil_softmax_pool_workspace_bytes(mlen, D, nseg)
    ws = _ws(wsb, h.device)
    big = STAMPS is not None and N * D >= (1 << 24)
    if big:
        _stamp("b", "softmax_pool_fwd", (N, D, nseg), 4.0 * N * D + 12.0 * N)
    if hpl is not None:
        _lib.check(L.advmil_softmax_pool_fwd_planes(_p(s), _p(hpl.hi), _p(hpl.lo), hpl.hi.stride(0), N, D, nseg,
                                                    _p(None if seg is None else seg.ptr), mlen, _p(A), _p(pooled), _p(ws), wsb, _stream()),
                   "softmax_pool_fwd_planes")
    else:
        _lib.check(L.advmil_softmax_pool_fwd(_p(s), _p(h), h.stride(0), N, D, nseg, _p(None if seg is None else seg.ptr), mlen, _p(A),
                                             _p(pooled), _p(ws), wsb, _stream()), "softmax_pool_fwd")
    if big:
        _stamp("e", "softmax_pool_fwd", (N, D, nseg), 4.0 * N * D + 12.0 * N)
    return A, pooled


def softmax_pool_mean(s, h, N, D, seg=None):
    L = _lib.lib()
    nseg = 1 if seg is None else seg.nseg
    mlen = N if seg is None else seg.max_len
    A = torch.empty(N, dtype=torch.float32, device=h.device)
    pooled = torch.empty(nseg, D, dtype=torch.float32, device=h.device)
    mean = torch.empty(nseg, D, dtype=torch.float32, device=h.device)
    wsb = L.advmil_softmax_pool_mean_workspace_bytes(mlen, D, nseg)
    ws = _ws(wsb, h.device)
    _lib.check(L.advmil_softmax_pool_mean_fwd(_p(s), _p(h), h.stride(0), N, D, nseg, _p(None if seg is None else seg.ptr), mlen, _p(A),
                                              _p(pooled), _p(mean), _p(ws), wsb, _stream()), "softmax_pool_mean_fwd")
    return A, pooled, mean


def softmax_pool_bwd(dpooled, dA, A, h, N, D, seg=None, hpl=None):
    L = _lib.lib()
    nseg = 1 if seg is None else seg.nseg
    mlen = N if seg is None else seg.max_len
    ds = torch.empty(N, dtype=torch.float32, device=h.device)
    wsb = L.advmil_softmax_pool_workspace_bytes(mlen, D, nseg)
    ws = _ws(wsb, h.device)
    if hpl is not None:
        _lib.check(L.advmil_softmax_pool_bwd_planes(_p(dpooled), _p(dA), _p(A), _p(hpl.hi), _p(hpl.lo), hpl.hi.stride(0), N, D, nseg,
                                                    _p(None if seg is None else seg.ptr), mlen, _p(ds), _p(ws), wsb, _stream()),
                   "softmax_pool_bwd_planes")
    else:
        _lib.check(L.advmil_softmax_pool_bwd(_p(dpooled), _p(dA), _p(A), _p(h), h.stride(0), N, D, nseg,
                                             _p(None if seg is None else seg.ptr), mlen, _p(ds), _p(ws), wsb, _stream()),
                   "softmax_pool_bwd")
    return ds


def dropout_planes(pl, M, N, p, seed, sid, rng_row=None, gate=None):
    out = Planes.alloc((M, N), pl.hi.device)
    out.fp32_stale = True
    bits = torch.empty(M, N // 32, dtype=torch.int32, device=pl.hi.device)
    gb = None
    if gate is not None:
        gb = (torch.empty(M, N // 32, dtype=torch.int32, device=pl.hi.device), torch.empty(M, N // 32, dtype=torch.int32, device=pl.hi.device))
    _lib.check(_lib.lib().advmil_dropout_planes(_p(pl.hi), _p(pl.lo), M, N, float(p), _p(seed), sid, _p(rng_row), _p(out.hi), _p(out.lo),
                                                _p(bits), 0.0 if gate is None else float(gate[0]), 0 if gate is None else int(gate[1]),
                                                0 if gate is None else int(gate[2]), _p(None if gb is None else gb[0]),
                                                _p(None if gb is None else gb[1]), _stream()), "dropout_planes")
    return (out, bits, gb) if gate is not None else (out, bits)


def planes_f32(pl):
    return pl.hi.float().add_(pl.lo)


def gate_bwd(ab, ds, wc, N, D, p=0.0, seed=None, stream_a=0, stream_b=0, dwc=None, dbc=None, dbias=None, rng_row=None, planes=None,
             planes_only=False, pair32=False):
    L = _lib.lib()
    dev = ab.device
    acc = dwc is not None
    dG = None if (planes_only and planes is not None) else torch.empty(N, 2 * D, dtype=torch.float32, device=dev)
    if not acc:
        dwc = torch.empty(D, dtype=torch.float32, device=dev)
        dbc = torch.empty(1, dtype=torch.float32, device=dev)
        dbias = torch.empty(2 * D, dtype=torch.float32, device=dev)
    wsb = L.advmil_gate_bwd_workspace_bytes(N, D)
    ws = _ws(wsb, dev)
    sd = seed if p > 0.0 else None
    _lib.check(L.advmil_gate_bwd(_p(ab), _p(ds), _p(wc), p, _p(sd), stream_a, stream_b, N, D, _p(dG), _p(dwc), _p(dbc),
                                 _p(dbias), 1 if acc else 0, _p(rng_row if sd is not None else None),
                                 _p(None if planes is None else planes.hi), _p(None if planes is None else planes.lo), 1 if pair32 else 0,
                                 _p(ws), wsb, _stream()), "gate_bwd")
    return dG, dwc, dbc, dbias


def act_dropout_bwd(dy, y, act, M, N, p=0.0, seed=None, stream_id=0, want_bias=True, db_out=None, rng_row=None, planes=None,
                    planes_only=False, bits=None):
    L = _lib.lib()
    dpre = None if (planes_only and planes is not None) else torch.empty(M, N, dtype=torch.float32, device=dy.device)
    acc = db_out is not None
    db = db_out if acc else (torch.empty(N, dtype=torch.float32, device=dy.device) if want_bias else None)
    need = acc or want_bias
    wsb = L.advmil_colsum_workspace_bytes(M, N) if need else 0
    ws = _ws(wsb, dy.device) if need else None
    sd = seed if p > 0.0 else None
# ... 235 lines not shown
                                                 1 if acc_b else 0, _p(dx), K, _p(ws), wsb, _stream()), f"small_linear_bwd[{M}x{N}x{K}]")
            return (dx, None if (dW is None or acc_w) else dW.reshape(wshape), None if (db is None or acc_b) else db,
                    None, None, None, None, None, None, None, None, None)
        if act == ACT_NONE and p <= 0.0:
            ent = DY_PLANES.pop(dy) if ctx.wants_dy_planes else None
            if ent is not None and ent[1] == (M, N) and need_w:
                dpl, xpl0 = ent[0], ctx.xpl
                if ctx.gW is not None:
                    gemm(None, x, False, False, N, K, M, out=ctx.gW.view(N, K), ldc=K, accumulate=True, a_planes=dpl, b_planes=xpl0)
                    return None, None, None, None, None, None, None, None, None, None, None, None
                dW = gemm(None, x, False, False, N, K, M, a_planes=dpl, b_planes=xpl0).reshape(wshape)
                return None, dW, None, None, None, None, None, None, None, None, None, None
            if ctx.wants_dy_planes and DY_PLANES.pending((M, N)):
                raise RuntimeError("advmil_amd: a gradient written as operand planes only did not reach the layer that asked for it "
                                   "(autograd re-wrapped the token tensor?)")
            dpre = dy
            if need_b:
                db = colsum(dy, M, N, out=ctx.gb)
        else:
            ent = DY_PLANES.pop(dy) if ctx.act_fusable else None
            if ent is not None and ent[1] == (M, N) and ent[2] == "dpre":
                dpl, xpl0 = ent[0], ctx.xpl
                if ctx.gW is not None:
                    gemm(None, x, False, False, N, K, M, out=ctx.gW.view(N, K), ldc=K, accumulate=True, a_planes=dpl, b_planes=xpl0)
                    return None, None, None, None, None, None, None, None, None, None, None, None
                dW = gemm(None, x, False, False, N, K, M, a_planes=dpl, b_planes=xpl0).reshape(wshape)
                return None, dW, None, None, None, None, None, None, None, None, None, None
            xpl0 = ctx.xpl if ((DW_PLANES or (ctx.xpl is not None and ctx.xpl.fp32_stale)) and get_gemm_mode() == "bf16x3") else None
            only = (DG_PLANES_ONLY and need_w and not need_x and xpl0 is not None and M >= 4096 and N % 8 == 0
                    and pre_a_tile_ok(gemm_plan(N, K, M, False, False)[0], False, False, True))
            dpl = Planes.alloc((M, N), dy.device) if only else None
            if getattr(ctx, "ypl", None) is not None:
                y = planes_f32(ctx.ypl)
            dpre, db = act_dropout_bwd(dy, y, act, M, N, p, seed, sid, want_bias=need_b, db_out=ctx.gb if need_b else None, rng_row=rr,
                                       planes=dpl, planes_only=only)
            if only:
                if ctx.gW is not None:
                    gemm(None, x, False, False, N, K, M, out=ctx.gW.view(N, K), ldc=K, accumulate=True, a_planes=dpl, b_planes=xpl0)
                    return None, None, (None if ctx.gb is not None else db), None, None, None, None, None, None, None, None, None
                dW = gemm(None, x, False, False, N, K, M, a_planes=dpl, b_planes=xpl0).reshape(wshape)
                return None, dW, (None if ctx.gb is not None else db), None, None, None, None, None, None, None, None, None
        dW = None
        if need_w:
            xpl = ctx.xpl if ((DW_PLANES or (ctx.xpl is not None and ctx.xpl.fp32_stale)) and get_gemm_mode() == "bf16x3") else None
            if xpl is None and is_bf16_slab(x):
                x = as_f32(x)
            if ctx.gW is not None:
                gemm(dpre, x, False, False, N, K, M, out=ctx.gW.view(N, K), ldc=K, accumulate=True, b_planes=xpl)
            else:
                dW = gemm(dpre, x, False, False, N, K, M, b_planes=xpl).reshape(wshape)
        dx = gemm(dpre, W2, True, False, M, K, N) if need_x else None
        return dx, dW, (None if ctx.gb is not None else db), None, None, None, None, None, None, None, None, None


class ForwardMemo:

    def __init__(self):
        self.mode, self.token, self.rows_ptr, self.store = None, None, None, {}
        self.derived, self.ln = {}, {}

    def begin(self, mode, token, rows):
        if token != self.token:
            self.store.clear(); self.derived.clear(); self.ln.clear()
        self.mode, self.token, self.rows_ptr = mode, token, rows.data_ptr()

    def knows(self, x):
        return self.mode is not None and (x.data_ptr() == self.rows_ptr or (MEMO_CHAIN and x.data_ptr() in self.derived))

    def end(self, clear=False):
        self.mode = None
        if clear:
            self.store.clear(); self.derived.clear(); self.ln.clear()


MEMO = ForwardMemo()
MEMO_CHAIN = os.environ.get("ADVMIL_MEMO_CHAIN", "1") != "0"
MEMO_MIN_ROWS = int(os.environ.get("ADVMIL_MEMO_MIN_ROWS", "4096"))


PREFILL = {}
TWO_LAYERS = os.environ.get("ADVMIL_TWO_LAYERS", "1") != "0"


def prefill_two_layers(X, layer1, layer2):
    (W1, b1, a1, emit1), (W2, b2, a2, _) = layer1, layer2
    if not TWO_LAYERS or X.dim() != 2 or not X.is_contiguous():
        return False
    M, K = X.shape
    W1m, W2m = W1.reshape(W1.shape[0], -1), W2.reshape(W2.shape[0], -1)
    if W2m.shape[1] != K or W1m.shape[1] != K or not gemm_two_layers_ok(M, W1m.shape[0], W2m.shape[0], K):
        return False
    xpl, p1, p2 = planes_of(X), weight_planes(W1), weight_planes(W2)
    if xpl is None or p1 is None or p2 is None:
        return False
    emit = bool(emit1) and bool(gemm_plan_planes(M, 2 * W1m.shape[0], W1m.shape[0]))
    only = bool(emit and H_PLANES_ONLY and a1 == "relu" and W1m.shape[0] % 32 == 0)
    with torch.no_grad():
        y1, y2, cpl = gemm_two_layers(X, xpl, W1m.detach(), Planes(p1.hi.reshape(W1m.shape), p1.lo.reshape(W1m.shape)),
                                      None if b1 is None else b1.detach(), _ACT[a1],
                                      W2m.detach(), Planes(p2.hi.reshape(W2m.shape), p2.lo.reshape(W2m.shape)),
                                      None if b2 is None else b2.detach(), _ACT[a2], emit, y1_planes_only=only)
    if only:
        y1._advmil_planes, y1._advmil_planes_only = cpl, True
    PREFILL[(X.data_ptr(), tuple(X.shape), W1.data_ptr(), W1._version, _ACT[a1])] = (y1, cpl)
    PREFILL[(X.data_ptr(), tuple(X.shape), W2.data_ptr(), W2._version, _ACT[a2])] = (y2, None)
    return True


def linear_act(x, W, b, act="none", p=0.0, rng=None, tag="", emit_planes=False, gate_sites=None):
    lead = x.shape[:-1]
    x2 = x if x.dim() == 2 else x.reshape(-1, x.shape[-1])
    sid, seed, rr = 0, None, None
    if p > 0.0:
        rng = rng or default_rng(x.device)
        N = W.shape[0]
        sid, seed, rr = rng.site(tag, (x2.shape[0], N), p), rng.seed, rng.row_map(x2.shape[0], tag)
    memo = MEMO if (MEMO.knows(x2) and x2.shape[0] >= MEMO_MIN_ROWS and (not x2.requires_grad or x2.data_ptr() != MEMO.rows_ptr)) else None
    key = (x2.data_ptr(), tuple(x2.shape), W.data_ptr(), W._version, act) if memo is not None else None
    y0 = None
    pre_planes = None
    if PREFILL and p <= 0.0:
        pf = PREFILL.pop((x2.data_ptr(), tuple(x2.shape), W.data_ptr(), W._version, _ACT[act]), None)
        if pf is not None:
            y0, pre_planes = pf
    if y0 is None and memo is not None and memo.mode == "replay":
        y0 = memo.store.pop(key, None)
        if y0 is not None:
            y0.record_stream(torch.cuda.current_stream())
    xpl = wpl = None
    if y0 is not None and p <= 0.0 and emit_planes:
        emit_planes = False
    big = x2.shape[0] >= 4096 and get_gemm_mode() == "bf16x3"
    stale = bool(getattr(x2, "_advmil_fp32_stale", False))
    if stale and (planes_of(x2) is None or get_gemm_mode() != "bf16x3"):
        raise RuntimeError("advmil_amd: a step slab staged as operand planes only reached a layer without its planes")
    if (y0 is None and big and (gemm_plan_planes(x2.shape[0], W.shape[0], x2.shape[1]) or (GENERIC_PLANES and planes_of(x2) is not None))) or stale:
        xpl, wpl = planes_of(x2), weight_planes(W)
        if wpl is not None:
            wpl = Planes(wpl.hi.reshape(W.shape[0], -1), wpl.lo.reshape(W.shape[0], -1))
    if is_bf16_slab(x2) and get_gemm_mode() != "bf16x3":
        x2 = as_f32(x2)
    emit = bool(emit_planes) and big and bool(gemm_plan_planes(x2.shape[0], 2 * W.shape[0], W.shape[0]))
    if emit_planes == "only":
        emit = "only" if (big and (act == "none" or not torch.is_grad_enabled()) and p <= 0.0 and y0 is None and W.shape[0] % 8 == 0
                          and ATTN_QKV_PLANES and (act == "none" or emit)) else (emit if act != "none" else False)
    LinearActFn.gate_request = ((float(gate_sites[0]), gate_sites[1], gate_sites[2], rng) if (gate_sites is not None and FUSED_GATE_TRAIN
                                and p > 0.0 and gate_sites[0] > 0.0 and torch.is_grad_enabled()) else None)
    LinearActFn.last_gate = None
    y = LinearActFn.apply(x2, W, b, _ACT[act], float(p), seed, sid, y0, rr, xpl, wpl, emit)
    LinearActFn.gate_request = None
    cpl, LinearActFn.last_planes = LinearActFn.last_planes, None
    if pre_planes is not None and cpl is None:
        cpl = pre_planes
    if memo is not None and memo.mode == "record" and p <= 0.0 and not torch.is_grad_enabled():
        memo.store[key] = y
        memo.derived[y.data_ptr()] = y
    out = y if len(lead) == 1 else y.reshape(*lead, y.shape[-1])
    if cpl is not None:
        out._advmil_planes = cpl
        if emit == "only" or cpl.fp32_stale:
            out._advmil_planes_only = True
    if LinearActFn.last_wants_dy_planes:
        out._advmil_wants_dy_planes = True
    LinearActFn.last_wants_dy_planes = False
    if LinearActFn.last_act_fusable is not None and out.requires_grad:
        out._advmil_act_fusable = LinearActFn.last_act_fusable + (LinearActFn.last_maskbits,)
    LinearActFn.last_act_fusable = None
    LinearActFn.last_maskbits = None
    if LinearActFn.last_gate is not None:
        out._advmil_gate = LinearActFn.last_gate
        LinearActFn.last_gate = None
    return out


def linear_act_any(x, W, b, act="none", p=0.0, rng=None, tag=""):
    K, N = W.shape[1], W.shape[0]
    if x.dim() != 2 or not x.is_cuda:
        raise RuntimeError("advmil_amd: linear layers run on 2-D HIP tensors only (no CPU / eager fallback)")
    if K % 4 == 0 and N % 4 == 0:
        return linear_act(x, W, b, act, p, rng, tag)
    pk, pn = (-K) % 4, (-N) % 4
    xp = torch.nn.functional.pad(x, (0, pk)) if pk else x
    Wp = torch.nn.functional.pad(W, (0, pk, 0, pn)) if (pk or pn) else W
    bp = None if b is None else (torch.nn.functional.pad(b, (0, pn)) if pn else b)
    y = linear_act(xp.contiguous(), Wp.contiguous(), bp, act)[:, :N]
    if p > 0.0:
        y = dropout(y.contiguous(), p, rng or default_rng(x.device), tag)
    return y


class GatedAttnPoolFn(torch.autograd.Function):

    @staticmethod
    def forward(ctx, h, Wa, ba, Wb, bb, wc, bc, p, seed, sa, sb, seg, nograd=False, rr=None, hpl=None, act_fuse=None, gate=None):
        _chk(h, "h")
        h = h.contiguous()
        N, D = h.shape
        ctx.act_fuse = act_fuse
        ctx.pair32 = False
        wcv = wc.detach().reshape(-1)
        stale = hpl is not None and hpl.fp32_stale
        ppl = hpl if stale else None
        if FUSED_GATE_SCORE and p <= 0.0 and N >= 4096 and nograd:
            Wi, bi, wipl = gate_interleave(Wa.detach(), ba.detach(), Wb.detach(), bb.detach(), D, planes=hpl is not None)
            s = gate_partial_sum(gemm(h, Wi, True, True, N, 2 * D, D, bias=bi, gate_wc=wcv, a_planes=hpl, b_planes=wipl), bc.detach())
            A, pooled = softmax_pool(s, h, N, D, seg, ppl)
            ctx.mark_non_differentiable(s)
            return pooled, A, s
        gs = [_arena_grad(t) for t in (Wa, ba, Wb, bb, wc, bc)]
        arena_ok = all(g is not None for g in gs) and _adjacent(gs[0], gs[2]) and _adjacent(gs[1], gs[3])
        if (gate is not None and FUSED_GATE_TRAIN and p > 0.0 and hpl is not None and arena_ok and N % 256 == 0 and D % 64 == 0
                and get_gemm_mode() == "bf16x3" and gemm_plan_planes(N, 2 * D, D) and gemm_plan_tn_planes(2 * D, D, N)[1] > 1
                and gemm_plan_planes(N, D, 2 * D)):
            Wp, bp, wppl = gate_interleave(Wa.detach(), ba.detach(), Wb.detach(), bb.detach(), D, planes=True, pair32=True)
            ab, part = gemm(h, Wp, True, True, N, 2 * D, D, bias=bp, gate_wc=wcv, drop_p=p, a_planes=hpl, b_planes=wppl, gate_bits=gate)
            s = gate_partial_sum(part, bc.detach())
            A, pooled = softmax_pool(s, h, N, D, seg, ppl)
            ctx.save_for_backward(h, Wp, ab, A, wcv)
            ctx.hpl, ctx.wabpl, ctx.pair32 = hpl, wppl, True
            ctx.cfg = (p, seed, sa, sb, N, D, wc.shape, seg, rr)
            ctx.arena = (gs[0].as_strided((2 * D, D), (D, 1), gs[0].storage_offset()),
                         gs[1].as_strided((2 * D,), (1,), gs[1].storage_offset()), gs[4].view(-1), gs[5])
            ctx.mark_non_differentiable(s)
            ctx.set_materialize_grads(False)
            return pooled, A, s
        Wab, _ = _stack2(Wa, Wb, D, D)
        bab, _ = _stack2(ba, bb, D, 0)
        wabpl = None
        if hpl is not None:
            pa_, pb_ = weight_planes(Wa), weight_planes(Wb)
            if pa_ is not None and pb_ is not None and _adjacent(pa_.hi, pb_.hi, 2) and _adjacent(pa_.lo, pb_.lo, 2):
                wabpl = Planes(pa_.hi.as_strided((2 * D, D), (D, 1), pa_.hi.storage_offset()),
                               pa_.lo.as_strided((2 * D, D), (D, 1), pa_.lo.storage_offset()))
            if wabpl is None and stale:
                wabpl = split_planes(Wab.detach().contiguous())
        ab = gemm(h, Wab, True, True, N, 2 * D, D, bias=bab, act0=ACT_TANH, act1=ACT_SIGMOID, act_split=D,
                  a_planes=hpl if wabpl is not None else None, b_planes=wabpl)
        s = gate_score(ab, wcv, bc, N, D, p, seed, sa, sb, rr)
        A, pooled = softmax_pool(s, h, N, D, seg, ppl)
        ctx.save_for_backward(h, Wab, ab, A, wcv)
        ctx.hpl = hpl
        ctx.wabpl = wabpl
        ctx.cfg = (p, seed, sa, sb, N, D, wc.shape, seg, rr)
        ctx.arena = None
        if arena_ok:
            ctx.arena = (gs[0].as_strided((2 * D, D), (D, 1), gs[0].storage_offset()),
                         gs[1].as_strided((2 * D,), (1,), gs[1].storage_offset()), gs[4].view(-1), gs[5])
        ctx.mark_non_differentiable(s)
        ctx.set_materialize_grads(False)
        return pooled, A, s

    @staticmethod
    def backward(ctx, dpooled, dA, _ds_unused):
        h, Wab, ab, A, wcv = ctx.saved_tensors
        p, seed, sa, sb, N, D, wcshape, seg, rr = ctx.cfg
        pair32 = bool(getattr(ctx, "pair32", False))
        nseg = 1 if seg is None else seg.nseg
        dpooled = (torch.zeros(nseg, D, dtype=torch.float32, device=h.device) if dpooled is None
                   else dpooled.contiguous().reshape(nseg, D))
        dA_ = None if dA is None else dA.contiguous()
        stale = ctx.hpl is not None and ctx.hpl.fp32_stale
        ds = softmax_pool_bwd(dpooled, dA_, A, h, N, D, seg, ctx.hpl if stale else None)
        need_h = ctx.needs_input_grad[0]
        gpl = None
        dh_tile = gemm_plan_planes(N, D, 2 * D) if (need_h and USE_PLANES and get_gemm_mode() == "bf16x3") else 0
        dh_nt = bool(dh_tile and DH_NT_FUSED and ctx.act_fuse is not None and ctx.act_fuse[2] is not None
                     and getattr(ctx, "wabpl", None) is not None and int(_lib.lib().advmil_gemm_f32_colsum_rows(dh_tile, N, D)) > 0)
        only = (DG_PLANES_ONLY and USE_PLANES and get_gemm_mode() == "bf16x3" and N >= 4096 and (2 * D) % 8 == 0
                and pre_a_tile_ok(gemm_plan(2 * D, D, N, False, False)[0], False, False)
                and (not need_h or pre_a_tile_ok(gemm_plan(N, D, 2 * D, True, False)[0], True, False)))
        if only and gpl is None:
            gpl = Planes.alloc((N, 2 * D), h.device)
        if ctx.arena is not None:
            gWab, gbab, gwc, gbc = ctx.arena
            dG, _, _, _ = gate_bwd(ab, ds, wcv, N, D, p, seed, sa, sb, dwc=gwc, dbc=gbc, dbias=gbab, rng_row=rr, planes=gpl, planes_only=only,
                                   pair32=pair32)
        else:
            dG, dwc, dbc, dbias = gate_bwd(ab, ds, wcv, N, D, p, seed, sa, sb, rng_row=rr, planes=gpl, planes_only=only)
        dh = None
        fuse = ctx.act_fuse if (need_h and only and ctx.act_fuse is not None) else None
        if fuse is not None and stale and fuse[2] is None:
            fuse = None
        wtpl = None
        if fuse is not None and dh_nt:
            nrow = int(_lib.lib().advmil_gemm_f32_colsum_rows(dh_tile, N, D))
            tile = dh_tile
            wtpl = planes_transposed(ctx.wabpl)
        elif fuse is not None:
            tile = gemm_plan(N, D, 2 * D, True, False)[0]
            nrow = int(_lib.lib().advmil_gemm_f32_colsum_rows(tile, N, D)) if pre_a_tile_ok(tile, True, False) else 0
            if nrow <= 0:
                fuse = None
        if fuse is not None:
            p1, gb1, mbits = fuse
            dpl = Planes.alloc((N, D), h.device)
            cws = _ws(nrow * D * 4, h.device) if gb1 is not None else None
            if wtpl is not None:
                gemm(None, None, True, True, N, D, 2 * D, rowv=A, colv=dpooled, rowseg=None if seg is None else seg.rowseg, a_planes=gpl,
                     b_planes=wtpl, maskbits=mbits, mask_scale=1.0 / (1.0 - p1) if p1 > 0.0 else 1.0, c_planes=dpl, c_planes_only=True,
                     colsum=cws, tile=tile)
            else:
                gemm(None, Wab, True, False, N, D, 2 * D, rowv=A, colv=dpooled, rowseg=None if seg is None else seg.rowseg, a_planes=gpl,
                     maskref=h if mbits is None else None, maskbits=mbits, mask_scale=1.0 / (1.0 - p1) if p1 > 0.0 else 1.0, c_planes=dpl,
                     c_planes_only=True, colsum=cws, tile=tile)
            if gb1 is not None:
                _lib.check(_lib.lib().advmil_merge_partials(_p(cws), nrow, D, D, _p(gb1), 1, _stream()), "merge_partials")
            dh = torch.empty(N, D, dtype=torch.float32, device=h.device)
            DY_PLANES.put(dh, dpl, (N, D), "dpre")
        elif need_h:
            if only:
                dh = gemm(None, Wab, True, False, N, D, 2 * D, rowv=A, colv=dpooled, rowseg=None if seg is None else seg.rowseg, a_planes=gpl)
            else:
                dh = gemm(dG, Wab, True, False, N, D, 2 * D, rowv=A, colv=dpooled, rowseg=None if seg is None else seg.rowseg)
        nones = (None,) * 10
        apl = gpl if only else None
        if ctx.arena is not None:
            bpl = ctx.hpl if (stale or (apl is not None and gemm_plan_tn_planes(2 * D, D, N)[0])) else None
            if pair32 and (apl is None or bpl is None):
                raise RuntimeError("advmil_amd: the pair-block gate backward needs dG and h as operand planes")
            gemm(dG, h, False, False, 2 * D, D, N, out=gWab, ldc=D, accumulate=True, a_planes=apl, b_planes=bpl, c_rows_pair32=pair32)
            return (dh, None, None, None, None, None, None) + nones
        bpl = ctx.hpl if (stale or (apl is not None and gemm_plan_tn_planes(2 * D, D, N)[0])) else None
        dWab = gemm(dG, h, False, False, 2 * D, D, N, a_planes=apl, b_planes=bpl)
        return (dh, dWab[:D], dbias[:D], dWab[D:], dbias[D:], dwc.reshape(wcshape), dbc) + nones


def gated_attn_pool(h, Wa, ba, Wb, bb, wc, bc, p=0.0, rng=None, tag="", seg=None):
    sa = sb = 0
    seed = rr = None
    gate = None
    if p > 0.0:
        rng = rng or default_rng(h.device)
        pre = getattr(h, "_advmil_gate", None)
        if pre is not None and pre[4] == float(p):
            sa, sb, gate = pre[0], pre[1], (pre[2], pre[3])
            seed, rr = rng.seed, pre[5]
        else:
            sa = rng.site(tag + "att_a", tuple(h.shape), p)
            sb = rng.site(tag + "att_b", tuple(h.shape), p)
            seed, rr = rng.seed, rng.row_map(h.shape[0], tag + "att_a")
    nograd = not torch.is_grad_enabled() or not any(t.requires_grad for t in (h, Wa, ba, Wb, bb, wc, bc))
    hpl = planes_of(h) if (h.shape[0] >= 4096 and h.is_contiguous() and get_gemm_mode() == "bf16x3"
                           and gemm_plan_planes(h.shape[0], 2 * h.shape[1], h.shape[1])) else None
    if getattr(h, "_advmil_planes_only", False):
        hpl = planes_of(h)
        if hpl is None or not hpl.fp32_stale:
            raise RuntimeError("advmil_amd: a planes-only activation reached the gated-attention pool without its planes")
    pooled, A, s = GatedAttnPoolFn.apply(h, Wa, ba, Wb, bb, wc, bc, float(p), seed, sa, sb, seg, nograd, rr, hpl,
                                         getattr(h, "_advmil_act_fusable", None), gate)
    return (pooled[0] if seg is None else pooled), A, s


class LNReLUMean16Fn(torch.autograd.Function):

    @staticmethod
    def forward(ctx, y, gamma, beta, eps, ycol=None, dy_planes=False, dup=1, memo=None):
        _chk(y, "y")
        y = y.contiguous()
        N, d = y.shape
        ctx.dup = dup
        if memo is not None:
            emb, mean, rstd = memo
            epl = None
        else:
            epl = None
            emb, mean, rstd = ln_relu_mean16_fwd(y, gamma, beta, N, d, eps, planes=epl, dup=dup)
        LNReLUMean16Fn.last_stats = (mean, rstd)
        LNReLUMean16Fn.last_planes = epl
        ctx.save_for_backward(y, gamma.detach(), beta.detach(), mean, rstd)
        gg, gb = _arena_grad(gamma), _arena_grad(beta)
# ... 505 lines not shown
        out = torch.empty(3, dtype=torch.float32, device=pred.device)
        gp, gf = torch.empty_like(pred_c), torch.empty_like(fake_c)
        t_c, e_c = t.contiguous().reshape(-1), e.contiguous().reshape(-1)
        _lib.check(_lib.lib().advmil_gan_g_loss(_p(pred_c), _p(t_c), _p(e_c), _p(vis), _p(fake_c), pred_c.numel(), alpha, gamma, l2,
                                                coef, inv_nf, inv_nv, _p(out), _p(gp), _p(gf), _stream()), "gan_g_loss")
        ctx.save_for_backward(gp, gf)
        ctx.shapes = (shape, fake.shape)
        ctx.mark_non_differentiable(out)
        ctx.set_materialize_grads(False)
        return out[0], out

    @staticmethod
    def backward(ctx, go, _):
        gp, gf = ctx.saved_tensors
        if go is None:
            return (None,) * 12
        if ctx.root:
            return (gp.reshape(ctx.shapes[0]), gf.reshape(ctx.shapes[1])) + (None,) * 10
        return ((gp * go).reshape(ctx.shapes[0]), (gf * go).reshape(ctx.shapes[1])) + (None,) * 10


def gan_g_loss(pred, fake, t, e, vis_mask, alpha, gamma, norm, coef, n_fake, n_vis, root=False):
    return GanGLossFn.apply(pred, fake, t, e, vis_mask, float(alpha), float(gamma), 1 if norm == "l2" else 0, float(coef),
                            1.0 / float(n_fake), (1.0 / float(n_vis)) if n_vis > 0 else 0.0, root)


class SkinnyLinearFn(torch.autograd.Function):

    @staticmethod
    def forward(ctx, x, W, b, act):
        x = x.contiguous()
        W2 = W.detach().reshape(W.shape[0], -1).contiguous()
        B, K = x.shape
        N = W2.shape[0]
        y = torch.empty(B, N, dtype=torch.float32, device=x.device)
        _lib.check(_lib.lib().advmil_skinny_linear_fwd(_p(x), _p(W2), _p(b), B, K, N, act, _p(y), _stream()), "skinny_linear_fwd")
        ctx.save_for_backward(x, W2, y)
        ctx.cfg = (act, B, K, N, W.shape, b is not None)
        ctx.gW, ctx.gb = _arena_grad(W), _arena_grad(b)
        return y

    @staticmethod
    def backward(ctx, dy):
        x, W2, y = ctx.saved_tensors
        act, B, K, N, wshape, has_b = ctx.cfg
        dy = dy.contiguous()
        need_x, need_w, need_b = ctx.needs_input_grad[0], ctx.needs_input_grad[1], has_b and ctx.needs_input_grad[2]
        dx = torch.empty(B, K, dtype=torch.float32, device=dy.device) if need_x else None
        arena = need_w and ctx.gW is not None and (not need_b or ctx.gb is not None)
        if arena:
            dW, db = ctx.gW, (ctx.gb if need_b else None)
        else:
            dW = torch.empty(N, K, dtype=torch.float32, device=dy.device) if need_w else None
            db = torch.empty(N, dtype=torch.float32, device=dy.device) if need_b else None
        _lib.check(_lib.lib().advmil_skinny_linear_bwd(_p(x), _p(W2), _p(y), _p(dy), B, K, N, act, _p(dx), _p(dW), _p(db),
                                                       1 if arena else 0, _stream()), "skinny_linear_bwd")
        if arena:
            return dx, None, None, None
        return dx, (None if dW is None else dW.reshape(wshape)), db, None


def skinny_linear(x, W, b, act="none"):
    return SkinnyLinearFn.apply(x, W, b, _ACT[act])


def gate_interleave(Wa, ba, Wb, bb, D, planes=False, pair32=False):
    Wa, Wb, ba, bb = (t.contiguous() for t in (Wa, Wb, ba, bb))
    dev = Wa.device
    Wi = torch.empty(2 * D, D, dtype=torch.float32, device=dev)
    bi = torch.empty(2 * D, dtype=torch.float32, device=dev)
    pl = Planes.alloc((2 * D, D), dev) if planes else None
    _lib.check(_lib.lib().advmil_gate_interleave(_p(Wa), _p(Wb), _p(ba), _p(bb), D, _p(Wi), _p(None if pl is None else pl.hi),
                                                 _p(None if pl is None else pl.lo), _p(bi), 1 if pair32 else 0, _stream()), "gate_interleave")
    return Wi, bi, pl


def gate_partial_sum(partial, bc=None):
    partial = partial.contiguous()
    N, npart = partial.shape
    s = torch.empty(N, dtype=torch.float32, device=partial.device)
    _lib.check(_lib.lib().advmil_gate_partial_sum(_p(partial), npart, _p(None if bc is None else bc.reshape(-1)), N, _p(s), _stream()),
               "gate_partial_sum")
    return s


class PrjHeadFn(torch.autograd.Function):

    @staticmethod
    def forward(ctx, u, t, src, W, b):
        u, t = u.contiguous(), t.contiguous()
        B, d = u.shape
        src_ = None if src is None else src.contiguous()
        w = None if W is None else W.detach().reshape(-1).contiguous()
        out = torch.empty(B, 1, dtype=torch.float32, device=u.device)
        _lib.check(_lib.lib().advmil_prj_head_fwd(_p(u), _p(t), _p(src_), _p(w), _p(None if b is None else b.detach()), B, d, _p(out),
                                                  _stream()), "prj_head_fwd")
        ctx.save_for_backward(u, t, src_, w)
        ctx.cfg = (B, d, None if W is None else W.shape, b is not None)
        ctx.gW, ctx.gb = _arena_grad(W), _arena_grad(b)
        return out

    @staticmethod
    def backward(ctx, dout):
        u, t, src, w = ctx.saved_tensors
        B, d, wshape, has_b = ctx.cfg
        dout = dout.contiguous()
        nu, nt, ns, nw = ctx.needs_input_grad[0], ctx.needs_input_grad[1], src is not None and ctx.needs_input_grad[2], \
            src is not None and ctx.needs_input_grad[3]
        nb = src is not None and has_b and ctx.needs_input_grad[4]
        new = lambda: torch.empty(B, d, dtype=torch.float32, device=dout.device)
        du, dt, ds = (new() if nu else None), (new() if nt else None), (new() if ns else None)
        arena = (nw or nb) and (not nw or ctx.gW is not None) and (not nb or ctx.gb is not None)
        if arena:
            dw, db = (ctx.gW if nw else None), (ctx.gb if nb else None)
        else:
            dw = torch.empty(d, dtype=torch.float32, device=dout.device) if nw else None
            db = torch.empty(1, dtype=torch.float32, device=dout.device) if nb else None
        _lib.check(_lib.lib().advmil_prj_head_bwd(_p(dout), _p(u), _p(t), _p(src), _p(w), B, d, _p(du), _p(dt), _p(ds), _p(dw), _p(db),
                                                  1 if arena else 0, _stream()), "prj_head_bwd")
        if arena:
            return du, dt, ds, None, None
        return du, dt, ds, (None if dw is None else dw.reshape(wshape)), db


def prj_head(u, t, src=None, W=None, b=None):
    return PrjHeadFn.apply(u, t, src, W, b)


DTAIL = os.environ.get("ADVMIL_DTAIL", "1") != "0"


class TailSpec:
    __slots__ = ("x", "y", "prj_w", "prj_b", "prj_src", "seed", "rr")

    def __init__(self, x, y, prj_w, prj_b, prj_src, seed, rr):
        self.x, self.y, self.prj_w, self.prj_b, self.prj_src, self.seed, self.rr = x, y, prj_w, prj_b, prj_src, seed, rr

    def params(self):
        out = []
        for (W, b, _, _, _) in self.x + self.y:
            out += [W, b]
        return out + [self.prj_w, self.prj_b]


def dtail_ok(B, spec):
    if not DTAIL or B > 32 or not (1 <= len(spec.x) <= _lib.TAIL_MAXL) or not (1 <= len(spec.y) <= _lib.TAIL_MAXL):
        return False
    for (W, b, _, _, _) in spec.x + spec.y:
        if W.dim() != 2 or max(W.shape) > 256 or W.dtype != torch.float32 or not W.is_cuda or not W.is_contiguous():
            return False
    if spec.x[-1][0].shape[0] != spec.y[-1][0].shape[0]:
        return False
    for p in spec.params():
        if p is not None and p.requires_grad and _arena_grad(p) is None:
            return False
    return True


def _fill_tail(dt, B, spec, ys_x, ys_y, xin, tin, u, slots):
    dt.B, dt.nx, dt.ny, dt.prj_src = B, len(spec.x), len(spec.y), spec.prj_src
    dt.xin, dt.tin = xin.data_ptr(), tin.data_ptr()
    dt.u = None if u is None else u.data_ptr()
    k = 0
    for arr, layers, ys in ((dt.x, spec.x, ys_x), (dt.y, spec.y, ys_y)):
        for i, ((W, b, act, p, sid), yb) in enumerate(zip(layers, ys)):
            L = arr[i]
# ... 306 lines not shown
```

### advmil_amd/optim.py

```python
import torch

from . import ops


def create_optimizer(args, model, filter_bias_and_bn=True):
    if args.opt.lower().split("_")[-1] != "adam":
        raise NotImplementedError(f"opt_netG={args.opt}: the AdvMIL configs use adam")
    wd = args.weight_decay or 0.0
    kw = {}
    if getattr(args, "opt_eps", None) is not None:
        kw["eps"] = args.opt_eps
    if getattr(args, "opt_betas", None) is not None:
        kw["betas"] = args.opt_betas
    return FlatAdam(model, lr=args.lr, weight_decay=wd, filter_bias_and_bn=bool(wd and filter_bias_and_bn), **kw)


class FlatAdam(torch.optim.Optimizer):
    def __init__(self, model, lr=1e-3, betas=(0.9, 0.999), eps=1e-8, weight_decay=0.0, filter_bias_and_bn=False, l1_coef=0.0):
        named = [(n, p) for n, p in model.named_parameters() if p.requires_grad]
        if not named:
            raise ValueError("no parameters")
        dev = named[0][1].device
        if dev.type != "cuda":
            raise RuntimeError("FlatAdam runs the fused HIP Adam kernel: move the model to the GPU first")
        if filter_bias_and_bn:
            no_decay = [(n, p) for n, p in named if p.dim() == 1 or n.endswith(".bias")]
            decay = [(n, p) for n, p in named if not (p.dim() == 1 or n.endswith(".bias"))]
            groups = [{"params": [p for _, p in no_decay], "weight_decay": 0.0},
                      {"params": [p for _, p in decay], "weight_decay": weight_decay}]
        else:
            groups = [{"params": [p for _, p in named], "weight_decay": weight_decay}]
        ordered = ([(n, p) for n, p in named if p.dim() == 1 or n.endswith(".bias")]
                   + [(n, p) for n, p in named if not (p.dim() == 1 or n.endswith(".bias"))])
        super().__init__(groups, dict(lr=lr, betas=betas, eps=eps, weight_decay=weight_decay))
        self.l1_coef = float(l1_coef)
        self.names = [n for n, _ in ordered]
        offs, total = [], 0
        for _, p in ordered:
            offs.append(total)
            total += (p.numel() + 7) // 8 * 8
        self.flat_param = torch.zeros(total, dtype=torch.float32, device=dev)
        self.flat_grad = torch.zeros(total, dtype=torch.float32, device=dev)
        ops.ARENA_STORAGES.add(self.flat_grad.untyped_storage().data_ptr())
        self.flat_m = torch.zeros(total, dtype=torch.float32, device=dev)
        self.flat_v = torch.zeros(total, dtype=torch.float32, device=dev)
        self.flat_wd = torch.zeros(total, dtype=torch.float32, device=dev)
        self.step_t = torch.zeros(1, dtype=torch.int32, device=dev)

        self.planes = ops.Planes.alloc((total,), dev)
        self.planes.hi.zero_(); self.planes.lo.zero_()
        self._views = []
        with torch.no_grad():
            for (n, p), o in zip(ordered, offs):
                k = p.numel()
                self.flat_param[o:o + k].copy_(p.reshape(-1))
                p.data = self.flat_param[o:o + k].view(p.shape)
                p.grad = self.flat_grad[o:o + k].view(p.shape)
                p._arena_grad = p.grad
                p._arena_owner = self
                self._views.append((p, o, k))
            for g in self.param_groups:
                for p in g["params"]:
                    o, k = next((o, k) for q, o, k in self._views if q is p)
                    self.flat_wd[o:o + k] = g["weight_decay"]
                    self.state[p] = {"step": torch.zeros((), dtype=torch.float32), "exp_avg": self.flat_m[o:o + k].view(p.shape),
                                     "exp_avg_sq": self.flat_v[o:o + k].view(p.shape)}
        self._has_wd = bool(self.flat_wd.abs().max().item() > 0)
        self.refresh_planes()

    def refresh_planes(self):
        ops.split_planes(self.flat_param, out=self.planes)
        for p, o, k in self._views:
            p._advmil_planes = (self, p._version, ops.Planes(self.planes.hi[o:o + k].view(p.shape), self.planes.lo[o:o + k].view(p.shape)))

    _grad_clean = False
    _clean_version = -1
    capture_assumes_clean = False

    def mark_grad_dirty(self):
        self._grad_clean = False

    def mark_grad_clean(self):
        self._grad_clean, self._clean_version = True, self.flat_grad._version

    def grad_is_clean(self):
        return bool(self._grad_clean and self.flat_grad._version == self._clean_version)

    def zero_grad(self, set_to_none: bool = False):
        if torch.cuda.is_current_stream_capturing():
            if not self.capture_assumes_clean:
                self.flat_grad.zero_()
        elif self.grad_is_clean():
            self._grad_clean = False
        else:
            self.flat_grad.zero_()
            self._grad_clean = False
        for p, o, k in self._views:
            if p.grad is None or p.grad.data_ptr() != self.flat_grad.data_ptr() + 4 * o:
                p.grad = self.flat_grad[o:o + k].view(p.shape)
                p._arena_grad = p.grad

    @torch.no_grad()
    def step(self, closure=None, grad_scale=1.0, tick=True, abs_partial=None, clear_grad=False):
        g0 = self.param_groups[0]
        b1, b2 = g0["betas"]
        self.n_updates = getattr(self, "n_updates", 0) + 1
        ops.adam_step(self.flat_param, self.flat_grad, self.flat_m, self.flat_v, self.flat_wd if self._has_wd else None,
                      self.step_t, g0["lr"], b1, b2, g0["eps"], grad_scale, self.l1_coef, planes=self.planes, tick=tick,
                      abs_partial=abs_partial, clear_grad=clear_grad)
        if not torch.cuda.is_current_stream_capturing():
            if clear_grad:
                self.mark_grad_clean()
            else:
                self._grad_clean = False

    def state_dict(self):
        n = float(self.step_t.item())
        for st in self.state.values():
            st["step"] = torch.tensor(n)
        return super().state_dict()

    def load_state_dict(self, sd):
        super().load_state_dict(sd)
        step = 0
        with torch.no_grad():
            for p, o, k in self._views:
                st = self.state[p]
                self.flat_m[o:o + k].copy_(st["exp_avg"].reshape(-1))
                self.flat_v[o:o + k].copy_(st["exp_avg_sq"].reshape(-1))
                st["exp_avg"] = self.flat_m[o:o + k].view(p.shape)
                st["exp_avg_sq"] = self.flat_v[o:o + k].view(p.shape)
                step = int(st["step"])
            self.step_t.fill_(step)
            for g in self.param_groups:
                for p in g["params"]:
                    o, k = next((o, k) for q, o, k in self._views if q is p)
                    self.flat_wd[o:o + k] = g["weight_decay"]
        self._has_wd = bool(self.flat_wd.abs().max().item() > 0)
        self.refresh_planes()
```

### include/advmil_hip.h

```cpp
#ifndef ADVMIL_HIP_H
#define ADVMIL_HIP_H
#include <stddef.h>
#include <stdint.h>

#ifdef __cplusplus
extern "C" {
#endif

typedef void* advmil_stream_t;

enum { ADVMIL_ACT_NONE = 0, ADVMIL_ACT_RELU = 1, ADVMIL_ACT_TANH = 2, ADVMIL_ACT_SIGMOID = 3 };

int advmil_version(void);

typedef struct {
  const float* bias;
  int act0, act1, act_split;
  float drop_p;
  const uint64_t* seed;
  uint64_t stream_id;
  const float* rowv;
  const float* colv;
  const int32_t* rowseg;
  const float* maskref;
  int ldmask;
  float mask_scale;
  int accumulate;
  float alpha;
  const void* a_hi;
  const void* a_lo;
  const void* b_hi;
  const void* b_lo;
  void* c_hi;
  void* c_lo;
  const float* gate_wc;
  float* gate_out;
  int gate_np;
  const int64_t* rng_row;
  float* c2;
  int64_t ldc2;
  int64_t n_split;
  const float* bias2;
  float* colsum;
  const uint32_t* maskbits;
  int64_t ldbits;
  const uint32_t* gate_bits_a;
  const uint32_t* gate_bits_b;
  int64_t ldgbits;
  int c_rows_pair32;
} advmil_epilogue_t;

size_t advmil_gemm_f32_workspace_bytes(int64_t M, int64_t N, int splits);
int advmil_gemm_f32(int a_kc, int b_kc, int64_t M, int64_t N, int64_t K, const float* A, int64_t lda,
                    const float* B, int64_t ldb, float* C, int64_t ldc, const advmil_epilogue_t* epi,
                    int splits, void* ws, size_t ws_bytes, advmil_stream_t stream);
int advmil_split_planes(const float* src, int64_t n, void* hi, void* lo, advmil_stream_t stream);
int advmil_gate_interleave(const float* Wa, const float* Wb, const float* ba, const float* bb, int D, float* Wi, void* Wi_hi, void* Wi_lo,
                           float* bi, int pair32, advmil_stream_t stream);
int advmil_gate_partial_sum(const float* partial, int np, const float* bc, int64_t N, float* s, advmil_stream_t stream);
int advmil_gemm_f32_gate_blocks(int tile, int64_t N);
int64_t advmil_gemm_f32_colsum_rows(int tile, int64_t M, int64_t N);
int advmil_merge_partials(const float* partial, int nblk, int64_t stride, int64_t ncols, float* out, int accumulate, advmil_stream_t stream);
int advmil_set_gemm_mode(int mode);
int advmil_get_gemm_mode(void);
int advmil_gemm_f32_plan(int64_t M, int64_t N, int64_t K, int* tile, int* splits);
int advmil_gemm_f32_plan_layout(int a_kc, int b_kc, int64_t M, int64_t N, int64_t K, int* tile, int* splits);
int advmil_gemm_f32_plan_planes(int a_kc, int b_kc, int64_t M, int64_t N, int64_t K, int* tile);
int advmil_gemm_f32_plan_tn_planes(int64_t M, int64_t N, int64_t K, int* tile, int* splits);
int advmil_gemm_f32_tiled(int a_kc, int b_kc, int64_t M, int64_t N, int64_t K, const float* A, int64_t lda,
                          const float* B, int64_t ldb, float* C, int64_t ldc, const advmil_epilogue_t* epi,
                          int splits, int tile, void* ws, size_t ws_bytes, advmil_stream_t stream);

int advmil_mha_fwd(const void* qkv_hi, const void* qkv_lo, int64_t Ltot, int nhead, int head_dim, int nseg, const int64_t* ptr,
                   int64_t max_len, float drop_p, const uint64_t* seed, uint64_t stream_id, const int64_t* rng_rowoff, float* out,
                   float* lse, advmil_stream_t stream);
int advmil_mha_fwd_lse(const void* qkv_hi, const void* qkv_lo, int64_t Ltot, int nhead, int head_dim, int nseg, const int64_t* ptr,
                       int64_t max_len, float drop_p, const uint64_t* seed, uint64_t stream_id, const int64_t* rng_rowoff, float* out,
                       const float* lse, advmil_stream_t stream);
size_t advmil_mha_bwd_workspace_bytes(int64_t Ltot, int nhead, int head_dim);
int advmil_mha_bwd(const void* qkv_hi, const void* qkv_lo, const float* out, const float* dout, const float* lse, int64_t Ltot,
                   int nhead, int head_dim, int nseg, const int64_t* ptr, int64_t max_len, float drop_p, const uint64_t* seed,
                   uint64_t stream_id, const int64_t* rng_rowoff, float* dqkv, void* ws, size_t ws_bytes, advmil_stream_t stream);
size_t advmil_mha_bwd1_workspace_bytes(int64_t Ltot, int nhead, int head_dim, int64_t max_len);
int advmil_mha_bwd1(const void* qkv_hi, const void* qkv_lo, const float* out, const float* dout, const float* lse, int64_t Ltot,
                    int nhead, int head_dim, int nseg, const int64_t* ptr, int64_t max_len, float drop_p, const uint64_t* seed,
                    uint64_t stream_id, const int64_t* rng_rowoff, float* dqkv, void* ws, size_t ws_bytes, advmil_stream_t stream);
int advmil_add_dropout_ln_fwd(const float* x, const float* o, const float* gamma, const float* beta, float eps, int64_t R,
                              int64_t d, float drop_p, const uint64_t* seed, uint64_t stream_id, const int64_t* rng_row, float* z,
                              float* y, float* mean, float* rstd, void* y_hi, void* y_lo, advmil_stream_t stream);
size_t advmil_add_dropout_ln_bwd_workspace_bytes(int64_t R, int64_t d);
int advmil_add_dropout_ln_bwd(const float* dy, const float* z, const float* gamma, const float* mean, const float* rstd, int64_t R,
                              int64_t d, float drop_p, const uint64_t* seed, uint64_t stream_id, const int64_t* rng_row, float* dx,
                              float* dob, float* dgamma, float* dbeta, int accumulate, void* ws, size_t ws_bytes,
                              advmil_stream_t stream);

int advmil_gate_score_fwd(const float* ab, const float* wc, const float* bc, float drop_p, const uint64_t* seed,
                          uint64_t stream_a, uint64_t stream_b, int64_t N, int64_t D, float* s, const int64_t* rng_row,
                          advmil_stream_t stream);
size_t advmil_softmax_pool_workspace_bytes(int64_t max_len, int64_t D, int nseg);
int advmil_softmax_pool_fwd(const float* s, const float* h, int64_t ldh, int64_t N, int64_t D, int nseg,
                            const int64_t* seg_ptr, int64_t max_len, float* A, float* pooled, void* ws, size_t ws_bytes,
                            advmil_stream_t stream);
size_t advmil_softmax_pool_mean_workspace_bytes(int64_t max_len, int64_t D, int nseg);
int advmil_softmax_pool_mean_fwd(const float* s, const float* h, int64_t ldh, int64_t N, int64_t D, int nseg, const int64_t* seg_ptr,
                                 int64_t max_len, float* A, float* pooled, float* mean, void* ws, size_t ws_bytes, advmil_stream_t stream);
int advmil_softmax_pool_bwd(const float* dpooled, const float* dA, const float* A, const float* h, int64_t ldh,
                            int64_t N, int64_t D, int nseg, const int64_t* seg_ptr, int64_t max_len, float* ds, void* ws,
                            size_t ws_bytes, advmil_stream_t stream);
int advmil_softmax_pool_fwd_planes(const float* s, const void* h_hi, const void* h_lo, int64_t ldh, int64_t N, int64_t D, int nseg,
                                   const int64_t* seg_ptr, int64_t max_len, float* A, float* pooled, void* ws, size_t ws_bytes,
                                   advmil_stream_t stream);
int advmil_softmax_pool_bwd_planes(const float* dpooled, const float* dA, const float* A, const void* h_hi, const void* h_lo, int64_t ldh,
                                   int64_t N, int64_t D, int nseg, const int64_t* seg_ptr, int64_t max_len, float* ds, void* ws,
                                   size_t ws_bytes, advmil_stream_t stream);
int advmil_dropout_planes(const void* in_hi, const void* in_lo, int64_t M, int64_t N, float drop_p, const uint64_t* seed, uint64_t stream_id,
                          const int64_t* rng_row, void* out_hi, void* out_lo, void* bits, float gate_p, uint64_t gate_stream_a,
                          uint64_t gate_stream_b, void* gate_bits_a, void* gate_bits_b, advmil_stream_t stream);
int advmil_seg_scale_rows(const float* dpooled, const float* A, const int32_t* rowseg, int64_t N, int64_t D, float* dh,
                          advmil_stream_t stream);
size_t advmil_gate_bwd_workspace_bytes(int64_t N, int64_t D);
int advmil_gate_bwd(const float* ab, const float* ds, const float* wc, float drop_p, const uint64_t* seed,
                    uint64_t stream_a, uint64_t stream_b, int64_t N, int64_t D, float* dG, float* dwc, float* dbc,
                    float* dbias, int accumulate, const int64_t* rng_row, void* dG_hi, void* dG_lo, int pair32, void* ws, size_t ws_bytes,
                    advmil_stream_t stream);

size_t advmil_colsum_workspace_bytes(int64_t M, int64_t N);
int advmil_act_dropout_bwd(const float* dy, const float* y, int act, float drop_p, const uint64_t* seed,
                           uint64_t stream_id, int64_t M, int64_t N, float* dpre, float* dbias, int accumulate,
                           const int64_t* rng_row, void* out_hi, void* out_lo, void* bits, void* ws, size_t ws_bytes,
                           advmil_stream_t stream);
int advmil_colsum(const float* x, int64_t M, int64_t N, float* out, int accumulate, void* ws, size_t ws_bytes,
                  advmil_stream_t stream);

int advmil_defer_sums(advmil_stream_t stream, int on);
int advmil_flush_sums(advmil_stream_t stream);
int advmil_pending_sums(advmil_stream_t stream);

int advmil_ln_relu_mean16_fwd(const float* y, const float* gamma, const float* beta, float eps, int64_t N, int64_t d,
                              float* emb, float* mean, float* rstd, void* emb_hi, void* emb_lo, int dup, advmil_stream_t stream);
size_t advmil_ln_relu_mean16_bwd_workspace_bytes(int64_t N, int64_t d);
int advmil_ln_relu_mean16_bwd(const float* demb, const float* y, const float* gamma, const float* beta,
                              const float* mean, const float* rstd, int64_t N, int64_t d, float* dy, float* dgamma,
                              float* dbeta, int accumulate, float* dycol, void* dy_hi, void* dy_lo, int dup, void* ws, size_t ws_bytes,
                              advmil_stream_t stream);

int advmil_ln_relu_fwd(const float* y, const float* gamma, const float* beta, float eps, int64_t N, int64_t d, float* out,
                       float* mean, float* rstd, advmil_stream_t stream);
size_t advmil_ln_relu_bwd_workspace_bytes(int64_t N, int64_t d);
int advmil_ln_relu_bwd(const float* dout, const float* y, const float* gamma, const float* beta, const float* mean,
                       const float* rstd, int64_t N, int64_t d, float* dy, float* dgamma, float* dbeta, int accumulate,
                       void* ws, size_t ws_bytes, advmil_stream_t stream);

int advmil_genconv_fwd(const float* x, const int32_t* rowptr_dst, const int32_t* col_src, const float* t, float eps, int64_t N,
                       int64_t C, float* out, float* lse, float* agg, advmil_stream_t stream);
size_t advmil_genconv_bwd_workspace_bytes(int64_t N, int64_t C);
int advmil_genconv_bwd(const float* dout, const float* x, const float* agg, const float* lse, const int32_t* rowptr_src,
                       const int32_t* col_dst, const float* t, float eps, int64_t N, int64_t C, float* dx, float* dt, void* ws,
                       size_t ws_bytes, advmil_stream_t stream);

int advmil_adam_blocks(int64_t n);
int advmil_adam_step(float* p, float* grad, float* m, float* v, const float* wd, int64_t n, float lr,
                     float beta1, float beta2, float eps, float grad_scale, float l1_coef, int32_t* step, void* p_hi, void* p_lo,
                     int tick, float* abs_partial, int clear_grad, advmil_stream_t stream);
int advmil_step_seed_tick(int32_t* step, int32_t* step2, uint64_t* seed, uint64_t inc, advmil_stream_t stream);
int advmil_abs_sum(const float* p, int64_t n, float* out, void* ws, size_t ws_bytes, advmil_stream_t stream);
size_t advmil_abs_sum_workspace_bytes(int64_t n);

int advmil_stage_bag(void* dst_rows, const void* src_rows, size_t rows_bytes, void* dst_hi, const void* src_hi, void* dst_lo,
                     const void* src_lo, size_t plane_bytes, advmil_stream_t stream);
int advmil_uniform_fill(float* out, int64_t n, const uint64_t* seed, uint64_t stream_id, const int64_t* rng_row, int64_t width,
                        advmil_stream_t stream);
int advmil_dropout_apply(const float* x, float* y, int64_t n, float p, const uint64_t* seed, uint64_t stream_id,
                         const int64_t* rng_row, int64_t width, advmil_stream_t stream);
int advmil_seed_advance(uint64_t* seed, uint64_t inc, advmil_stream_t stream);
int advmil_stamp_clock(int64_t* dst, advmil_stream_t stream);
int64_t advmil_clock_rate_khz(void);
int advmil_skinny_linear_fwd(const float* x, const float* W, const float* bias, int B, int K, int N, int act, float* y,
                             advmil_stream_t stream);
int advmil_skinny_linear_bwd(const float* x, const float* W, const float* y, const float* dy, int B, int K, int N, int act, float* dx,
                             float* dW, float* dbias, int accumulate, advmil_stream_t stream);
int advmil_small_linear_fwd(const float* x, int64_t ldx, const float* W, const float* bias, int M, int N, int K, int act, float drop_p,
                            const uint64_t* seed, uint64_t stream_id, const int64_t* rng_row, float* y, advmil_stream_t stream);
size_t advmil_small_linear_bwd_workspace_bytes(int M, int N);
int advmil_small_linear_bwd(const float* dy, const float* y, const float* x, int64_t ldx, const float* W, int M, int N, int K, int act,
                            float drop_p, const uint64_t* seed, uint64_t stream_id, const int64_t* rng_row, float* dW, int acc_w,
                            float* dbias, int acc_b, float* dx, int64_t lddx, void* ws, size_t ws_bytes, advmil_stream_t stream);
int advmil_prj_head_fwd(const float* u, const float* t, const float* src, const float* w, const float* bias, int B, int d, float* out,
                        advmil_stream_t stream);
int advmil_prj_head_bwd(const float* dout, const float* u, const float* t, const float* src, const float* w, int B, int d, float* du,
                        float* dt, float* dsrc, float* dw, float* dbias, int accumulate, advmil_stream_t stream);
#define ADVMIL_TAIL_MAXL 3
typedef struct {
  const float* W;
  const float* bias;
// ... 101 lines not shown
```

Before: 5715 bags/s.

## Fuse per-step weight prep into one kernel and fold gate partial sum into pooling

Adds a single step_weight_prep kernel that builds the interleaved and pair32 gate weight layouts, their bf16 hi/lo planes, the transposed planes and a concatenated two-layer weight stack in one launch. The results are cached by optimizer generation and capture epoch, so they are rebuilt only after weights change. A partials variant of the softmax pool kernel sums the gate GEMM partials plus bias inline, which removes the separate gate_partial_sum launch and a round trip of the score array through memory. The cost is extra cache-key bookkeeping and generation counters in the optimizer, plus a risk of stale weights if an invalidation path is missed.

```diff
diff --git a/advmil_amd/_lib.py b/advmil_amd/_lib.py
--- a/advmil_amd/_lib.py
+++ b/advmil_amd/_lib.py
@@ -51,6 +51,13 @@
                 ("hs", c_void_p), ("h2", c_void_p), ("pred", c_void_p), ("dpred", c_void_p), ("dx", c_void_p), ("lddx", c_int64),
                 ("dWr", c_void_p), ("dbr", c_void_p), ("dW0", c_void_p), ("db0", c_void_p), ("dW1", c_void_p), ("db1", c_void_p),
                 ("ws", c_void_p), ("ws_bytes", c_size_t)]
+
+
+class WeightPrep(ctypes.Structure):
+    _fields_ = [("w1_hi", c_void_p), ("w1_lo", c_void_p), ("w2_hi", c_void_p), ("w2_lo", c_void_p), ("N1", c_int64), ("N2", c_int64),
+                ("K", c_int64), ("cat_hi", c_void_p), ("cat_lo", c_void_p), ("Wa", c_void_p), ("Wb", c_void_p), ("ba", c_void_p),
+                ("bb", c_void_p), ("D", c_int32), ("Wi", c_void_p), ("wi_hi", c_void_p), ("wi_lo", c_void_p), ("bi", c_void_p),
+                ("Wp", c_void_p), ("wp_hi", c_void_p), ("wp_lo", c_void_p), ("bp", c_void_p), ("wpt_hi", c_void_p), ("wpt_lo", c_void_p)]
 
 
 SIGNATURES = {
@@ -62,6 +69,7 @@
     "advmil_stage_bag": (c_int, [c_void_p, c_void_p, c_size_t, c_void_p, c_void_p, c_void_p, c_void_p, c_size_t, c_void_p]),
     "advmil_gate_interleave": (c_int, [c_void_p, c_void_p, c_void_p, c_void_p, c_int, c_void_p, c_void_p, c_void_p, c_void_p, c_int, c_void_p]),
     "advmil_gate_partial_sum": (c_int, [c_void_p, c_int, c_void_p, c_int64, c_void_p, c_void_p]),
+    "advmil_step_weight_prep": (c_int, [ctypes.POINTER(WeightPrep), c_void_p]),
     "advmil_gemm_f32_gate_blocks": (c_int, [c_int, c_int64]),
     "advmil_gemm_f32_colsum_rows": (c_int64, [c_int, c_int64, c_int64]),
     "advmil_merge_partials": (c_int, [c_void_p, c_int, c_int64, c_int64, c_void_p, c_int, c_void_p]),
@@ -101,6 +109,8 @@
                                         c_int64, c_void_p, c_void_p, c_size_t, c_void_p]),
     "advmil_softmax_pool_fwd_planes": (c_int, [c_void_p, c_void_p, c_void_p, c_int64, c_int64, c_int64, c_int, c_void_p, c_int64, c_void_p,
                                                c_void_p, c_void_p, c_size_t, c_void_p]),
+    "advmil_softmax_pool_fwd_partials": (c_int, [c_void_p, c_int, c_void_p, c_void_p, c_void_p, c_void_p, c_int64, c_int64, c_int64, c_int, c_void_p,
+                                                 c_int64, c_void_p, c_void_p, c_void_p, c_size_t, c_void_p]),
     "advmil_softmax_pool_bwd_planes": (c_int, [c_void_p, c_void_p, c_void_p, c_void_p, c_void_p, c_int64, c_int64, c_int64, c_int, c_void_p,
                                                c_int64, c_void_p, c_void_p, c_size_t, c_void_p]),
     "advmil_dropout_planes": (c_int, [c_void_p, c_void_p, c_int64, c_int64, c_float, c_void_p, c_uint64, c_void_p, c_void_p, c_void_p, c_void_p,
diff --git a/advmil_amd/csrc/pool.hip b/advmil_amd/csrc/pool.hip
--- a/advmil_amd/csrc/pool.hip
+++ b/advmil_amd/csrc/pool.hip
@@ -317,11 +317,14 @@
   v1.w = __uint_as_float(a.w & 0xffff0000u) + __uint_as_float(b.w & 0xffff0000u);
 }
 
-template <bool MEAN, bool PL = false>
-__global__ __launch_bounds__(256) void pool_partial8_online_kernel(const float* __restrict__ s, const float* __restrict__ h, int64_t ldh,
+template <bool MEAN, bool PL = false, bool PART = false>
+__global__ __launch_bounds__(256) void pool_partial8_online_kernel(const float* __restrict__ s_in, const float* __restrict__ h, int64_t ldh,
                                                                    int64_t N, int64_t D, const int64_t* __restrict__ seg_ptr,
                                                                    float* __restrict__ partial, float* __restrict__ pstats, int rpb,
-                                                                   float* __restrict__ mpartial, const bf16raw* __restrict__ hlo = nullptr) {
+                                                                   float* __restrict__ mpartial, const bf16raw* __restrict__ hlo = nullptr,
+                                                                   const float* __restrict__ gpart = nullptr, int gnp = 0,
+                                                                   const float* __restrict__ gbc = nullptr, float* __restrict__ s_out = nullptr) {
+  const float* __restrict__ s = s_in;
   __shared__ __attribute__((aligned(16))) float red[2048];
   __shared__ float wts[512];
   __shared__ float wred[8];
@@ -335,6 +338,23 @@
   float* pst = pstats + ((int64_t)b * gridDim.x + blockIdx.x) * 2;
   float* prow = partial + ((int64_t)b * gridDim.x + blockIdx.x) * D;
   float* mrow = MEAN ? mpartial + ((int64_t)b * gridDim.x + blockIdx.x) * D : nullptr;
+  const float gb = (PART && gbc) ? gbc[0] : 0.f;
+  if constexpr (PART) {
+    if (blockIdx.x == 0 && (b == 0 || b == (int)gridDim.y - 1)) {
+      const int64_t o0 = b == 0 ? 0 : end, o1 = b == 0 ? beg : N;
+      for (int64_t n = o0 + tid; n < o1; n += 256) {
+        float a = 0.f;
+        for (int j = 0; j < gnp; ++j) a += gpart[n * gnp + j];
+        s_out[n] = a + gb;
+      }
+      if (b == 0 && gridDim.y == 1)
+        for (int64_t n = end + tid; n < N; n += 256) {
+          float a = 0.f;
+          for (int j = 0; j < gnp; ++j) a += gpart[n * gnp + j];
+          s_out[n] = a + gb;
+        }
+    }
+  }
   if (r0 >= end) {
     if (tid < (int)(D >> 2)) {
       *reinterpret_cast<float4*>(prow + tid * 4) = make_float4(0.f, 0.f, 0.f, 0.f);
@@ -346,7 +366,17 @@
   float mx = -INFINITY;
   for (int r = tid; r < rpb; r += 256) {
     const int64_t n = r0 + r;
-    const float v = n < end ? s[n] : -INFINITY;
+    float v = -INFINITY;
+    if constexpr (PART) {
+      if (n < end) {
+        float a = 0.f;
+        for (int j = 0; j < gnp; ++j) a += gpart[n * gnp + j];
+        v = a + gb;
+        s_out[n] = v;
+      }
+    } else {
+      v = n < end ? s[n] : -INFINITY;
+    }
     wts[r] = v;
     mx = fmaxf(mx, v);
   }
@@ -507,7 +537,7 @@
 
 static int softmax_pool_fwd_impl(const float* s, const float* h, int64_t ldh, int64_t N, int64_t D, int nseg, const int64_t* seg_ptr,
                                  int64_t max_len, float* A, float* pooled, float* mean, void* ws, size_t ws_bytes, hipStream_t stream,
-                                 const bf16raw* hlo = nullptr);
+                                 const bf16raw* hlo = nullptr, const float* gpart = nullptr, int gnp = 0, const float* gbc = nullptr);
 
 extern "C" int advmil_softmax_pool_fwd(const float* s, const float* h, int64_t ldh, int64_t N, int64_t D, int nseg,
                                        const int64_t* seg_ptr, int64_t max_len, float* A, float* pooled, void* ws,
@@ -523,6 +553,14 @@
                                (const bf16raw*)h_lo);
 }
 
+extern "C" int advmil_softmax_pool_fwd_partials(const float* partial, int np, const float* bc, float* s, const void* h, const void* h_lo,
+                                                int64_t ldh, int64_t N, int64_t D, int nseg, const int64_t* seg_ptr, int64_t max_len,
+                                                float* A, float* pooled, void* ws, size_t ws_bytes, advmil_stream_t stream_) {
+  if (!partial || np <= 0) return ADVMIL_EINVAL;
+  return softmax_pool_fwd_impl(s, (const float*)h, ldh, N, D, nseg, seg_ptr, max_len, A, pooled, nullptr, ws, ws_bytes, (hipStream_t)stream_,
+                               (const bf16raw*)h_lo, partial, np, bc);
+}
+
 static inline size_t pool_mean_offset_bytes(int64_t max_len, int64_t D, int nseg) {
   return (advmil_softmax_pool_workspace_bytes(max_len, D, nseg) + 15) / 16 * 16;
 }
@@ -541,7 +579,7 @@
 
 static int softmax_pool_fwd_impl(const float* s, const float* h, int64_t ldh, int64_t N, int64_t D, int nseg, const int64_t* seg_ptr,
                                  int64_t max_len, float* A, float* pooled, float* mean, void* ws, size_t ws_bytes, hipStream_t stream,
-                                 const bf16raw* hlo) {
+                                 const bf16raw* hlo, const float* gpart, int gnp, const float* gbc) {
   if (!s || !h || !A || !pooled || !ws || N <= 0 || D <= 0 || (D & 3) || D > 1024 || (ldh & 3)) return ADVMIL_EINVAL;
   if (ldh < D || ((uintptr_t)h & 15)) return ADVMIL_EINVAL;
   if (hlo && (((uintptr_t)hlo & 15) || (D & 7) || (ldh & 7) || D < 16 || mean)) return ADVMIL_EINVAL;
@@ -555,6 +593,7 @@
   const int nblk = (int)pool_nblk(max_len);
   if ((D & 7) == 0 && D >= 16 && nblk <= POOL_ONLINE_MAX_NBLK) {
     float* pstats = partial + (int64_t)nseg * nblk * D;
+    if (mean && gpart) return ADVMIL_EINVAL;
     if (mean) {
       float* mpartial = (float*)ws + pool_mean_offset_bytes(max_len, D, nseg) / sizeof(float);
       hipLaunchKernelGGL((pool_partial8_online_kernel<true, false>), dim3(nblk, nseg), dim3(256), 0, stream, s, h, ldh, N, D, seg_ptr, partial, pstats,
@@ -565,7 +604,13 @@
       ADVMIL_LAUNCH_CHECK();
       return ADVMIL_OK;
     }
-    if (hlo)
+    if (gpart && hlo)
+      hipLaunchKernelGGL((pool_partial8_online_kernel<false, true, true>), dim3(nblk, nseg), dim3(256), 0, stream, s, h, ldh, N, D, seg_ptr, partial,
+                         pstats, rows_per_block(max_len), (float*)nullptr, hlo, gpart, gnp, gbc, (float*)s);
+    else if (gpart)
+      hipLaunchKernelGGL((pool_partial8_online_kernel<false, false, true>), dim3(nblk, nseg), dim3(256), 0, stream, s, h, ldh, N, D, seg_ptr,
+                         partial, pstats, rows_per_block(max_len), (float*)nullptr, (const bf16raw*)nullptr, gpart, gnp, gbc, (float*)s);
+    else if (hlo)
       hipLaunchKernelGGL((pool_partial8_online_kernel<false, true>), dim3(nblk, nseg), dim3(256), 0, stream, s, h, ldh, N, D, seg_ptr, partial,
                          pstats, rows_per_block(max_len), (float*)nullptr, hlo);
     else
@@ -577,7 +622,7 @@
     ADVMIL_LAUNCH_CHECK();
     return ADVMIL_OK;
   }
-  if (mean || hlo) return ADVMIL_EINVAL;
+  if (mean || hlo || gpart) return ADVMIL_EINVAL;
   hipLaunchKernelGGL(softmax_stats_kernel, dim3(nseg), dim3(1024), 0, stream, s, N, seg_ptr, stats);
   ADVMIL_LAUNCH_CHECK();
   if ((D & 7) == 0 && D >= 16)
@@ -848,6 +893,75 @@
   int64_t blocks = (N + 255) / 256;
   if (blocks > 2048) blocks = 2048;
   hipLaunchKernelGGL(gate_partial_sum_kernel, dim3((unsigned)blocks), dim3(256), 0, (hipStream_t)stream_, partial, np, bc, N, s);
+  ADVMIL_LAUNCH_CHECK();
+  return ADVMIL_OK;
+}
+
+__global__ __launch_bounds__(256) void step_weight_prep_kernel(const advmil_weight_prep_t p, int64_t n_cat, int64_t n_gate, int64_t n_t) {
+  const int D = p.D, q4 = D >> 2;
+  const int64_t total = n_cat + n_gate + n_t;
+  for (int64_t e = (int64_t)blockIdx.x * 256 + threadIdx.x; e < total; e += (int64_t)gridDim.x * 256) {
+    if (e < n_cat) {
+      const int64_t k8 = p.K >> 3, r = e / k8, c = (e % k8) * 8;
+      const bf16raw* shi = r < p.N1 ? (const bf16raw*)p.w1_hi + r * p.K : (const bf16raw*)p.w2_hi + (r - p.N1) * p.K;
+      const bf16raw* slo = r < p.N1 ? (const bf16raw*)p.w1_lo + r * p.K : (const bf16raw*)p.w2_lo + (r - p.N1) * p.K;
+      *reinterpret_cast<uint4*>((bf16raw*)p.cat_hi + r * p.K + c) = *reinterpret_cast<const uint4*>(shi + c);
+      *reinterpret_cast<uint4*>((bf16raw*)p.cat_lo + r * p.K + c) = *reinterpret_cast<const uint4*>(slo + c);
+    } else if (e < n_cat + n_gate) {
+      const int64_t g = e - n_cat;
+      const int s = (int)(g / q4), c = (int)(g % q4) * 4;
+      const int br = s >= D, j = br ? s - D : s;
+      const float4 v = *reinterpret_cast<const float4*>((br ? p.Wb : p.Wa) + (int64_t)j * D + c);
+      uint2 hh, ll;
+      split4(v, hh, ll);
+      const int64_t oi = (int64_t)(2 * j + br) * D + c;
+      const int64_t op = (int64_t)(((j >> 5) << 6) | (br << 5) | (j & 31)) * D + c;
+      *reinterpret_cast<float4*>(p.Wi + oi) = v;
+      *reinterpret_cast<uint2*>((bf16raw*)p.wi_hi + oi) = hh;
+      *reinterpret_cast<uint2*>((bf16raw*)p.wi_lo + oi) = ll;
+      *reinterpret_cast<float4*>(p.Wp + op) = v;
+      *reinterpret_cast<uint2*>((bf16raw*)p.wp_hi + op) = hh;
+      *reinterpret_cast<uint2*>((bf16raw*)p.wp_lo + op) = ll;
+    } else {
+      const int64_t t = e - n_cat - n_gate;
+      const int c = (int)(t % D), r0 = (int)(t / D) * 8;
+      const int br = (r0 >> 5) & 1, j0 = ((r0 >> 6) << 5) | (r0 & 31);
+      const float* src = (br ? p.Wb : p.Wa) + (int64_t)j0 * D + c;
+      uint4 hh, ll;
+      split2(src[0], src[D], hh.x, ll.x);
+      split2(src[2 * (int64_t)D], src[3 * (int64_t)D], hh.y, ll.y);
+      split2(src[4 * (int64_t)D], src[5 * (int64_t)D], hh.z, ll.z);
+      split2(src[6 * (int64_t)D], src[7 * (int64_t)D], hh.w, ll.w);
+      *reinterpret_cast<uint4*>((bf16raw*)p.wpt_hi + (int64_t)c * 2 * D + r0) = hh;
+      *reinterpret_cast<uint4*>((bf16raw*)p.wpt_lo + (int64_t)c * 2 * D + r0) = ll;
+    }
+  }
+  if (blockIdx.x == 0)
+    for (int r = threadIdx.x; r < 2 * D; r += 256) {
+      p.bi[r] = (r & 1) ? p.bb[r >> 1] : p.ba[r >> 1];
+      const int j = ((r >> 6) << 5) | (r & 31);
+      p.bp[r] = ((r >> 5) & 1) ? p.bb[j] : p.ba[j];
+    }
+}
+extern "C" int advmil_step_weight_prep(const advmil_weight_prep_t* p, advmil_stream_t stream_) {
+  if (!p) return ADVMIL_EINVAL;
+  if (!p->Wa || !p->Wb || !p->ba || !p->bb || !p->Wi || !p->wi_hi || !p->wi_lo || !p->bi || !p->Wp || !p->wp_hi || !p->wp_lo || !p->bp
+      || !p->wpt_hi || !p->wpt_lo || p->D <= 0 || (p->D & 31))
+    return ADVMIL_EINVAL;
+  if (((uintptr_t)p->Wa | (uintptr_t)p->Wb | (uintptr_t)p->Wi | (uintptr_t)p->Wp | (uintptr_t)p->wpt_hi | (uintptr_t)p->wpt_lo) & 15) return ADVMIL_EINVAL;
+  if (((uintptr_t)p->wi_hi | (uintptr_t)p->wi_lo | (uintptr_t)p->wp_hi | (uintptr_t)p->wp_lo) & 7) return ADVMIL_EINVAL;
+  int64_t n_cat = 0;
+  if (p->cat_hi || p->cat_lo) {
+    if (!p->cat_hi || !p->cat_lo || !p->w1_hi || !p->w1_lo || !p->w2_hi || !p->w2_lo || p->N1 <= 0 || p->N2 <= 0 || p->K <= 0 || (p->K & 7))
+      return ADVMIL_EINVAL;
+    if (((uintptr_t)p->cat_hi | (uintptr_t)p->cat_lo | (uintptr_t)p->w1_hi | (uintptr_t)p->w1_lo | (uintptr_t)p->w2_hi | (uintptr_t)p->w2_lo) & 15)
+      return ADVMIL_EINVAL;
+    n_cat = (p->N1 + p->N2) * (p->K >> 3);
+  }
+  const int64_t D = p->D, n_gate = 2 * D * (D >> 2), n_t = D * (2 * D >> 3);
+  int64_t blocks = (n_cat + n_gate + n_t + 255) / 256;
+  if (blocks > 1024) blocks = 1024;
+  hipLaunchKernelGGL(step_weight_prep_kernel, dim3((unsigned)blocks), dim3(256), 0, (hipStream_t)stream_, *p, n_cat, n_gate, n_t);
   ADVMIL_LAUNCH_CHECK();
   return ADVMIL_OK;
 }
diff --git a/advmil_amd/graphed.py b/advmil_amd/graphed.py
--- a/advmil_amd/graphed.py
+++ b/advmil_amd/graphed.py
@@ -107,6 +107,13 @@
         self._st_d, self._st_g = h._st_d, h._st_g
 
     def _capture_graphs(self, pool):
+        ops.PREP_EPOCH += 1
+        try:
+            self._capture_graphs_epoch(pool)
+        finally:
+            ops.PREP_EPOCH += 1
+
+    def _capture_graphs_epoch(self, pool):
         h = self.h
         if self.site_base is not None:
             h.rng.counter = self.site_base
@@ -140,6 +147,8 @@
         if self._lrs() != self.lrs:
             self.segments, self.lrs = [], self._lrs()
             self._capture(0)
+        for opt in (self.h.optimizerD, self.h.optimizerG):
+            opt.generation += 1
         segs = self.segments
         if CLEAR_IN_ADAM:
             for opt in (self.h.optimizerD, self.h.optimizerG):
diff --git a/advmil_amd/model/model_handler.py b/advmil_amd/model/model_handler.py
--- a/advmil_amd/model/model_handler.py
+++ b/advmil_amd/model/model_handler.py
@@ -609,9 +609,13 @@
     @staticmethod
     def _prefill_static(netG, netD, bcb, X):
         bb = netG.backbone
+        gate = None
         if bcb == "abmil" and hasattr(bb, "attention_net"):
             fc = bb.attention_net[0]
             l1 = (fc.weight, fc.bias, "relu", True)
+            sc = bb.attention_net[3]
+            if hasattr(sc, "attention_a") and hasattr(sc, "attention_b"):
+                gate = (sc.attention_a[0].weight, sc.attention_a[0].bias, sc.attention_b[0].weight, sc.attention_b[0].bias)
         elif bcb == "patch" and hasattr(bb, "patch_embedding_layer") and hasattr(bb.patch_embedding_layer, "conv"):
             cv = bb.patch_embedding_layer.conv
             l1 = (cv.weight, cv.bias, "none", False)
@@ -620,7 +624,7 @@
         emb = getattr(getattr(netD, "net_pair_one", None), "embedding", None)
         if emb is None or not hasattr(emb, "conv"):
             return False
-        return ops.prefill_two_layers(X, l1, (emb.conv.weight, emb.conv.bias, "none", False))
+        return ops.prefill_two_layers(X, l1, (emb.conv.weight, emb.conv.bias, "none", False), gate=gate)
 
     def _gen_features(self, X, plan, xs):
         exts = [x[1] for x in xs] if self.bcb in ("cluster", "graph") else None
diff --git a/advmil_amd/ops.py b/advmil_amd/ops.py
--- a/advmil_amd/ops.py
+++ b/advmil_amd/ops.py
@@ -578,7 +578,7 @@
     return gemm_two_layers_tile(M, N1, N2, K) != 0
 
 
-def gemm_two_layers(x, xpl, W1, w1pl, b1, act1, W2, w2pl, b2, act2, emit_planes1=False, y1_planes_only=False):
+def gemm_two_layers(x, xpl, W1, w1pl, b1, act1, W2, w2pl, b2, act2, emit_planes1=False, y1_planes_only=False, wcat=None):
     M, K = x.shape
     N1, N2 = W1.shape[0], W2.shape[0]
 
@@ -588,8 +588,10 @@
         if hi.untyped_storage().data_ptr() != lo.untyped_storage().data_ptr() or d <= 0 or not hi.is_contiguous() or not lo.is_contiguous():
             return None
         return hi.as_strided((2, N, K), (d, K, 1), hi.storage_offset())
-    v1, v2 = pair(w1pl, N1), pair(w2pl, N2)
-    if v1 is not None and v2 is not None:
+    v1, v2 = (None, None) if wcat is not None else (pair(w1pl, N1), pair(w2pl, N2))
+    if wcat is not None:
+        pass
+    elif v1 is not None and v2 is not None:
         stk = torch.cat((v1, v2), dim=1)
         wcat = Planes(stk[0], stk[1])
     else:
@@ -684,10 +686,13 @@
         return self._div[key]
 
 
-def softmax_pool(s, h, N, D, seg=None, hpl=None):
+def softmax_pool(s, h, N, D, seg=None, hpl=None, partials=None):
+    want_s = partials is not None
     L = _lib.lib()
     nseg = 1 if seg is None else seg.nseg
     mlen = N if seg is None else seg.max_len
+    if partials is not None and not (D % 8 == 0 and D >= 16 and mlen <= (1 << 20)):
+        s, partials = gate_partial_sum(*partials), None
     A = torch.empty(N, dtype=torch.float32, device=h.device)
     pooled = torch.empty(nseg, D, dtype=torch.float32, device=h.device)
     wsb = L.advmil_softmax_pool_workspace_bytes(mlen, D, nseg)
@@ -695,7 +700,16 @@
     big = STAMPS is not None and N * D >= (1 << 24)
     if big:
         _stamp("b", "softmax_pool_fwd", (N, D, nseg), 4.0 * N * D + 12.0 * N)
-    if hpl is not None:
+    if partials is not None:
+        part, bc = partials
+        part = part.contiguous()
+        s = torch.empty(N, dtype=torch.float32, device=h.device)
+        hp = h if hpl is None else hpl.hi
+        _lib.check(L.advmil_softmax_pool_fwd_partials(_p(part), part.shape[1], _p(None if bc is None else bc.reshape(-1)), _p(s), _p(hp),
+                                                      _p(None if hpl is None else hpl.lo), hp.stride(0), N, D, nseg,
+                                                      _p(None if seg is None else seg.ptr), mlen, _p(A), _p(pooled), _p(ws), wsb, _stream()),
+                   "softmax_pool_fwd_partials")
+    elif hpl is not None:
         _lib.check(L.advmil_softmax_pool_fwd_planes(_p(s), _p(hpl.hi), _p(hpl.lo), hpl.hi.stride(0), N, D, nseg,
                                                     _p(None if seg is None else seg.ptr), mlen, _p(A), _p(pooled), _p(ws), wsb, _stream()),
                    "softmax_pool_fwd_planes")
@@ -704,6 +718,8 @@
                                              _p(pooled), _p(ws), wsb, _stream()), "softmax_pool_fwd")
     if big:
         _stamp("e", "softmax_pool_fwd", (N, D, nseg), 4.0 * N * D + 12.0 * N)
+    if want_s:
+        return A, pooled, s
     return A, pooled
 
 
@@ -1105,7 +1121,7 @@
 TWO_LAYERS = os.environ.get("ADVMIL_TWO_LAYERS", "1") != "0"
 
 
-def prefill_two_layers(X, layer1, layer2):
+def prefill_two_layers(X, layer1, layer2, gate=None):
     (W1, b1, a1, emit1), (W2, b2, a2, _) = layer1, layer2
     if not TWO_LAYERS or X.dim() != 2 or not X.is_contiguous():
         return False
@@ -1118,11 +1134,13 @@
         return False
     emit = bool(emit1) and bool(gemm_plan_planes(M, 2 * W1m.shape[0], W1m.shape[0]))
     only = bool(emit and H_PLANES_ONLY and a1 == "relu" and W1m.shape[0] % 32 == 0)
+    prep = StepWeightPrep.of(*gate, W1=W1, W2=W2) if (gate is not None and W1.dim() == 2 and W2.dim() == 2) else None
     with torch.no_grad():
         y1, y2, cpl = gemm_two_layers(X, xpl, W1m.detach(), Planes(p1.hi.reshape(W1m.shape), p1.lo.reshape(W1m.shape)),
                                       None if b1 is None else b1.detach(), _ACT[a1],
                                       W2m.detach(), Planes(p2.hi.reshape(W2m.shape), p2.lo.reshape(W2m.shape)),
-                                      None if b2 is None else b2.detach(), _ACT[a2], emit, y1_planes_only=only)
+                                      None if b2 is None else b2.detach(), _ACT[a2], emit, y1_planes_only=only,
+                                      wcat=None if prep is None else prep.stack())
     if only:
         y1._advmil_planes, y1._advmil_planes_only = cpl, True
     PREFILL[(X.data_ptr(), tuple(X.shape), W1.data_ptr(), W1._version, _ACT[a1])] = (y1, cpl)
@@ -1221,13 +1239,19 @@
         N, D = h.shape
         ctx.act_fuse = act_fuse
         ctx.pair32 = False
+        ctx.wtpl = None
         wcv = wc.detach().reshape(-1)
         stale = hpl is not None and hpl.fp32_stale
         ppl = hpl if stale else None
         if FUSED_GATE_SCORE and p <= 0.0 and N >= 4096 and nograd:
-            Wi, bi, wipl = gate_interleave(Wa.detach(), ba.detach(), Wb.detach(), bb.detach(), D, planes=hpl is not None)
-            s = gate_partial_sum(gemm(h, Wi, True, True, N, 2 * D, D, bias=bi, gate_wc=wcv, a_planes=hpl, b_planes=wipl), bc.detach())
-            A, pooled = softmax_pool(s, h, N, D, seg, ppl)
+            prep = StepWeightPrep.of(Wa, ba, Wb, bb)
+            if prep is not None:
+                Wi, bi, wipl = prep.gate(False)
+                wipl = wipl if hpl is not None else None
+            else:
+                Wi, bi, wipl = gate_interleave(Wa.detach(), ba.detach(), Wb.detach(), bb.detach(), D, planes=hpl is not None)
+            part = gemm(h, Wi, True, True, N, 2 * D, D, bias=bi, gate_wc=wcv, a_planes=hpl, b_planes=wipl)
+            A, pooled, s = softmax_pool(None, h, N, D, seg, ppl, partials=(part, bc.detach()))
             ctx.mark_non_differentiable(s)
             return pooled, A, s
         gs = [_arena_grad(t) for t in (Wa, ba, Wb, bb, wc, bc)]
@@ -1235,10 +1259,14 @@
         if (gate is not None and FUSED_GATE_TRAIN and p > 0.0 and hpl is not None and arena_ok and N % 256 == 0 and D % 64 == 0
                 and get_gemm_mode() == "bf16x3" and gemm_plan_planes(N, 2 * D, D) and gemm_plan_tn_planes(2 * D, D, N)[1] > 1
                 and gemm_plan_planes(N, D, 2 * D)):
-            Wp, bp, wppl = gate_interleave(Wa.detach(), ba.detach(), Wb.detach(), bb.detach(), D, planes=True, pair32=True)
+            prep = StepWeightPrep.of(Wa, ba, Wb, bb)
+            if prep is not None:
+                Wp, bp, wppl = prep.gate(True)
+                ctx.wtpl = prep.wpt
+            else:
+                Wp, bp, wppl = gate_interleave(Wa.detach(), ba.detach(), Wb.detach(), bb.detach(), D, planes=True, pair32=True)
             ab, part = gemm(h, Wp, True, True, N, 2 * D, D, bias=bp, gate_wc=wcv, drop_p=p, a_planes=hpl, b_planes=wppl, gate_bits=gate)
-            s = gate_partial_sum(part, bc.detach())
-            A, pooled = softmax_pool(s, h, N, D, seg, ppl)
+            A, pooled, s = softmax_pool(None, h, N, D, seg, ppl, partials=(part, bc.detach()))
             ctx.save_for_backward(h, Wp, ab, A, wcv)
             ctx.hpl, ctx.wabpl, ctx.pair32 = hpl, wppl, True
             ctx.cfg = (p, seed, sa, sb, N, D, wc.shape, seg, rr)
@@ -1308,7 +1336,7 @@
         if fuse is not None and dh_nt:
             nrow = int(_lib.lib().advmil_gemm_f32_colsum_rows(dh_tile, N, D))
             tile = dh_tile
-            wtpl = planes_transposed(ctx.wabpl)
+            wtpl = ctx.wtpl if ctx.wtpl is not None else planes_transposed(ctx.wabpl)
         elif fuse is not None:
             tile = gemm_plan(N, D, 2 * D, True, False)[0]
             nrow = int(_lib.lib().advmil_gemm_f32_colsum_rows(tile, N, D)) if pre_a_tile_ok(tile, True, False) else 0
@@ -1980,6 +2008,101 @@
     _lib.check(_lib.lib().advmil_gate_partial_sum(_p(partial), npart, _p(None if bc is None else bc.reshape(-1)), N, _p(s), _stream()),
                "gate_partial_sum")
     return s
+
+
+PREP_EPOCH = 0
+STEP_WEIGHT_PREP = True
+
+
+class StepWeightPrep:
+
+    def __init__(self, Wa, ba, Wb, bb, W1=None, W2=None):
+        self.gate_params, self.W1, self.W2 = (Wa, ba, Wb, bb), W1, W2
+        self.D = int(Wa.shape[0])
+        self._key_gate = self._key_stack = None
+        self.wi = self.wp = self.wpt = self.wcat = None
+
+    @staticmethod
+    def of(Wa, ba, Wb, bb, W1=None, W2=None):
+        if not (STEP_WEIGHT_PREP and USE_PLANES and get_gemm_mode() == "bf16x3"):
+            return None
+        D = Wa.shape[0]
+        own = getattr(Wa, "_arena_owner", None)
+        if (own is None or any(getattr(t, "_arena_owner", None) is not own for t in (ba, Wb, bb)) or D % 32 or tuple(Wa.shape) != (D, D)
+                or tuple(Wb.shape) != (D, D) or any((t.data_ptr() & 15) or not t.is_contiguous() for t in (Wa, Wb))):
+            return None
+        if W1 is not None:
+            if (getattr(W1, "_arena_owner", None) is not own or getattr(W2, "_arena_owner", None) is None or W1.shape[1] != W2.shape[1]
+                    or W1.shape[1] % 8 or weight_planes(W1) is None or weight_planes(W2) is None):
+                W1 = W2 = None
+        prep = getattr(Wa, "_advmil_prep", None)
+        if (prep is None or any(a is not b for a, b in zip(prep.gate_params, (Wa, ba, Wb, bb)))
+                or (W1 is not None and (prep.W1 is not W1 or prep.W2 is not W2))):
+            prep = StepWeightPrep(Wa, ba, Wb, bb, W1, W2)
+            Wa._advmil_prep = prep
+        return prep
+
+    def _keys(self):
+        ps = self.gate_params + (() if self.W1 is None else (self.W1, self.W2))
+        for t in ps:
+            weight_planes(t)
+        where = (PREP_EPOCH, bool(torch.cuda.is_current_stream_capturing()))
+        g = self.gate_params[0]._arena_owner
+        kg = where + (id(g), g.generation) + tuple(t.data_ptr() for t in self.gate_params)
+        if self.W1 is None:
+            return kg, None
+        d = self.W2._arena_owner
+        return kg, kg + (id(d), d.generation, self.W1.data_ptr(), self.W2.data_ptr())
+
+    def _build(self, kg, ks):
+        Wa, ba, Wb, bb = (t.detach() for t in self.gate_params)
+        D, dev = self.D, Wa.device
+        f = torch.empty(2 * (2 * D * D + 2 * D), dtype=torch.float32, device=dev)
+        Wi, Wp = f[:2 * D * D].view(2 * D, D), f[2 * D * D:4 * D * D].view(2 * D, D)
+        bi, bp = f[4 * D * D:4 * D * D + 2 * D], f[4 * D * D + 2 * D:]
+        wipl, wppl, wtpl = Planes.alloc((2 * D, D), dev), Planes.alloc((2 * D, D), dev), Planes.alloc((D, 2 * D), dev)
+        a = _lib.WeightPrep()
+        a.Wa, a.Wb, a.ba, a.bb, a.D = Wa.data_ptr(), Wb.data_ptr(), ba.data_ptr(), bb.data_ptr(), D
+        a.Wi, a.wi_hi, a.wi_lo, a.bi = Wi.data_ptr(), wipl.hi.data_ptr(), wipl.lo.data_ptr(), bi.data_ptr()
+        a.Wp, a.wp_hi, a.wp_lo, a.bp = Wp.data_ptr(), wppl.hi.data_ptr(), wppl.lo.data_ptr(), bp.data_ptr()
+        a.wpt_hi, a.wpt_lo = wtpl.hi.data_ptr(), wtpl.lo.data_ptr()
+        wcat = None
+        if ks is not None:
+            p1, p2 = weight_planes(self.W1), weight_planes(self.W2)
+            N1, N2, K = int(self.W1.shape[0]), int(self.W2.shape[0]), int(self.W1.shape[1])
+            wcat = Planes.alloc((N1 + N2, K), dev)
+            a.w1_hi, a.w1_lo, a.w2_hi, a.w2_lo = p1.hi.data_ptr(), p1.lo.data_ptr(), p2.hi.data_ptr(), p2.lo.data_ptr()
+            a.N1, a.N2, a.K = N1, N2, K
+            a.cat_hi, a.cat_lo = wcat.hi.data_ptr(), wcat.lo.data_ptr()
+        _lib.check(_lib.lib().advmil_step_weight_prep(ctypes.byref(a), _stream()), "step_weight_prep")
+        self.wi, self.wp, self.wpt, self.wcat = (Wi, bi, wipl), (Wp, bp, wppl), wtpl, wcat
+        self._key_gate, self._key_stack = kg, ks
+        self._bufs = [f] + [t for pl in (wipl, wppl, wtpl, wcat) if pl is not None for t in (pl.hi, pl.lo)]
+        self._built_on = _stream().value
+
+    def _reused(self):
+        if _stream().value != self._built_on and not torch.cuda.is_current_stream_capturing():
+            cur = torch.cuda.current_stream()
+            for t in self._bufs:
+                t.record_stream(cur)
+
+    def gate(self, pair32):
+        kg, ks = self._keys()
+        if kg != self._key_gate:
+            self._build(kg, ks)
+        else:
+            self._reused()
+        return self.wp if pair32 else self.wi
+
+    def stack(self):
+        kg, ks = self._keys()
+        if ks is None:
+            return None
+        if ks != self._key_stack or kg != self._key_gate:
+            self._build(kg, ks)
+        else:
+            self._reused()
+        return self.wcat
 
 
 class PrjHeadFn(torch.autograd.Function):
diff --git a/advmil_amd/optim.py b/advmil_amd/optim.py
--- a/advmil_amd/optim.py
+++ b/advmil_amd/optim.py
@@ -68,7 +68,10 @@
         self._has_wd = bool(self.flat_wd.abs().max().item() > 0)
         self.refresh_planes()
 
+    generation = 0
+
     def refresh_planes(self):
+        self.generation += 1
         ops.split_planes(self.flat_param, out=self.planes)
         for p, o, k in self._views:
             p._advmil_planes = (self, p._version, ops.Planes(self.planes.hi[o:o + k].view(p.shape), self.planes.lo[o:o + k].view(p.shape)))
@@ -105,6 +108,7 @@
         g0 = self.param_groups[0]
         b1, b2 = g0["betas"]
         self.n_updates = getattr(self, "n_updates", 0) + 1
+        self.generation += 1
         ops.adam_step(self.flat_param, self.flat_grad, self.flat_m, self.flat_v, self.flat_wd if self._has_wd else None,
                       self.step_t, g0["lr"], b1, b2, g0["eps"], grad_scale, self.l1_coef, planes=self.planes, tick=tick,
                       abs_partial=abs_partial, clear_grad=clear_grad)
diff --git a/include/advmil_hip.h b/include/advmil_hip.h
--- a/include/advmil_hip.h
+++ b/include/advmil_hip.h
@@ -58,6 +58,21 @@
 int advmil_gate_interleave(const float* Wa, const float* Wb, const float* ba, const float* bb, int D, float* Wi, void* Wi_hi, void* Wi_lo,
                            float* bi, int pair32, advmil_stream_t stream);
 int advmil_gate_partial_sum(const float* partial, int np, const float* bc, int64_t N, float* s, advmil_stream_t stream);
+typedef struct {
+  const void *w1_hi, *w1_lo, *w2_hi, *w2_lo;
+  int64_t N1, N2, K;
+  void *cat_hi, *cat_lo;
+  const float *Wa, *Wb, *ba, *bb;
+  int32_t D;
+  float* Wi;
+  void *wi_hi, *wi_lo;
+  float* bi;
+  float* Wp;
+  void *wp_hi, *wp_lo;
+  float* bp;
+  void *wpt_hi, *wpt_lo;
+} advmil_weight_prep_t;
+int advmil_step_weight_prep(const advmil_weight_prep_t* p, advmil_stream_t stream);
 int advmil_gemm_f32_gate_blocks(int tile, int64_t N);
 int64_t advmil_gemm_f32_colsum_rows(int tile, int64_t M, int64_t N);
 int advmil_merge_partials(const float* partial, int nblk, int64_t stride, int64_t ncols, float* out, int accumulate, advmil_stream_t stream);
@@ -110,6 +125,9 @@
 int advmil_softmax_pool_fwd_planes(const float* s, const void* h_hi, const void* h_lo, int64_t ldh, int64_t N, int64_t D, int nseg,
                                    const int64_t* seg_ptr, int64_t max_len, float* A, float* pooled, void* ws, size_t ws_bytes,
                                    advmil_stream_t stream);
+int advmil_softmax_pool_fwd_partials(const float* partial, int np, const float* bc, float* s, const void* h, const void* h_lo, int64_t ldh,
+                                     int64_t N, int64_t D, int nseg, const int64_t* seg_ptr, int64_t max_len, float* A, float* pooled,
+                                     void* ws, size_t ws_bytes, advmil_stream_t stream);
 int advmil_softmax_pool_bwd_planes(const float* dpooled, const float* dA, const float* A, const void* h_hi, const void* h_lo, int64_t ldh,
                                    int64_t N, int64_t D, int nseg, const int64_t* seg_ptr, int64_t max_len, float* ds, void* ws,
                                    size_t ws_bytes, advmil_stream_t stream);
```

Measured after the change: 5743 bags/s (median of 6 runs). No clear change (+0.5%).
